# galatolofederico/clip-glass

Hardware: AMD Instinct MI355X
Metric: candidate latents scored/sec (GAN→CLIP fitness), StyleGAN2_ffhq_d pop=64 (higher is better)
Workload: dtype f16; 1 GPU; StyleGAN2_ffhq_d: StyleGAN2 config-f 1024px G+D + CLIP ViT-B/32, pop=64 per GPU, batch_size=4, n_obj=2; pop_per_gpu=64, global_pop=64, batch_size=4, parallelism=population-shard x1, device=AMD Radeon Graphics (gfx950:sramecc+:xnack-), 256 CUs, hbm_gib=288

## Files before the change

### clip_glass_amd/csrc/common.h

```cpp
#pragma once
#include <hip/hip_runtime.h>
#include <stdint.h>

#include <atomic>
#include <mutex>
#include <stdio.h>
#include <stdlib.h>

typedef _Float16 half_t;
typedef _Float16 h2 __attribute__((ext_vector_type(2)));
typedef _Float16 h4 __attribute__((ext_vector_type(4)));
typedef _Float16 h8 __attribute__((ext_vector_type(8)));
typedef float f4 __attribute__((ext_vector_type(4)));
typedef float f16x __attribute__((ext_vector_type(16)));

#define GLASS_SQRT2 1.41421356237309504880f

__device__ __forceinline__ f16x mfma32(h8 a, h8 b, f16x c) {
    return __builtin_amdgcn_mfma_f32_32x32x16_f16(a, b, c, 0, 0, 0);
}
__device__ __forceinline__ int mfma32_row(int reg, int lane) { return (reg & 3) + 8 * (reg >> 2) + 4 * (lane >> 5); }
__device__ __forceinline__ void philox4x32_10(uint32_t c[4], uint32_t k0, uint32_t k1) {
#pragma unroll
    for (int i = 0; i < 10; ++i) {
// ... 18 lines not shown
    const int my = oy >> 1, mx = ox >> 1;
    const float wy0 = (oy & 1) ? 0.25f : 0.75f, wx0 = (ox & 1) ? 0.25f : 0.75f;
    float s = 0.f;
    s += ((my >= 1 && mx >= 1) ? wy0 * wx0 : 0.f) * t[0];
    s += (my >= 1 ? wy0 * (1.f - wx0) : 0.f) * t[1];
    s += (mx >= 1 ? (1.f - wy0) * wx0 : 0.f) * t[2];
    s += (1.f - wy0) * (1.f - wx0) * t[3];
    return s;
}

struct DevOnce {
    std::atomic<bool> done[32] = {};
    static int dev() {
        int d = 0;
        if (hipGetDevice(&d) != hipSuccess || d < 0 || d >= 32) return -1;
        return d;
    }
    bool first() const {
        const int d = dev();
        return d < 0 || !done[d].load(std::memory_order_acquire);
    }
    void set() {
        const int d = dev();
        if (d >= 0) done[d].store(true, std::memory_order_release);
    }
    template <class F> void run(F&& setup) {
        if (first()) {
            setup();
            set();
        }
    }
};
struct GlassDevProps { int cus, lds_optin; };
inline GlassDevProps glass_dev_props() {
    static std::atomic<int> cus[32] = {}, lds[32] = {};
    int d = 0;
    if (hipGetDevice(&d) != hipSuccess || d < 0 || d >= 32) d = 0;
    if (!cus[d].load()) {
        hipDeviceProp_t prop;
        if (hipGetDeviceProperties(&prop, d) == hipSuccess) {
            lds[d].store((int)prop.sharedMemPerBlockOptin > 0 ? (int)prop.sharedMemPerBlockOptin : (int)prop.sharedMemPerBlock);
            cus[d].store(prop.multiProcessorCount);
        }
    }
    return GlassDevProps{cus[d].load() > 0 ? cus[d].load() : 256, lds[d].load() > 0 ? lds[d].load() : 64 * 1024};
}
inline int glass_cu_count() { return glass_dev_props().cus; }
inline bool glass_lds_fits(int bytes) {
    const GlassDevProps dp = glass_dev_props();
    if (bytes <= dp.lds_optin) return true;
    static std::mutex mu;
    static int seen_dev[16], seen_bytes[16], n_seen = 0;
    int d = 0;
    (void)hipGetDevice(&d);
    std::lock_guard<std::mutex> lk(mu);
    for (int i = 0; i < n_seen; ++i)
        if (seen_dev[i] == d && seen_bytes[i] == bytes) return false;
    if (n_seen == 16) return false;
    seen_dev[n_seen] = d;
    seen_bytes[n_seen++] = bytes;
    if (n_seen == 16) fprintf(stderr, "libglass: further LDS refusals are not reported\n");
    fprintf(stderr, "libglass: device %d offers %d B of opt-in LDS per workgroup; a kernel family that needs %d B is refused and its "
                    "layers fall back to a slower kernel (expected on gfx950: 163840 B)\n", d, dp.lds_optin, bytes);
    return false;
}

#define GLASS_NOMINAL_POP 64

__device__ __forceinline__ float lrelu_sqrt2(float v) { return (v > 0.f ? v : 0.2f * v) * GLASS_SQRT2; }
struct ActK { float k1, k2; };
__device__ __forceinline__ ActK act_consts(int act, float s) {
    return ActK{(act == 1 ? GLASS_SQRT2 : 1.f) * s, (act == 1 ? 0.2f * GLASS_SQRT2 : act == 2 ? 0.f : 1.f) * s};
}
__device__ __forceinline__ f4 act_apply(f4 v, ActK k) { return __builtin_elementwise_max(v * k.k1, v * k.k2); }

struct ConvParams {
    const half_t* x;
    long long x_bstride;
    int B, H, W, Cin;
    int Hc, Wc;
    int KS, stride, pad;
    const half_t* w;
    const half_t* w_up;
    long long w_bstride;
    int Neff, Cout;
    int up;
    int Ho, Wo;
    const float* sn;
    int sn_stride;
    const half_t* sn16;
    const half_t* pre_shift16;
    const float* pre_shift;
    int in_up;
    const float* dscale;
    int ds_stride;
    const float* noise;
    float noise_strength;
    int batch_size;
    const float* bias;
    const float* shift;
    int act;
    const half_t* res;
    int res_cs;
    int res_up;
    float out_scale;
    const float* rgb_y;
    const float* rgb_w;
    const float* rgb_b;
    half_t* rgb_x_out;
    half_t* rgb_xs_out;
    const float* trgb_w;
    const float* trgb_b;
    const float* trgb_sn;
    int trgb_sn_stride;
    const float* trgb_smax;
    int trgb_smax_stride;
    const float* trgb_yprev;
    float* trgb_yout;
    float* rgb_tanh_out;
    float* trgb_part;
    const half_t* trgb_tab;
    half_t* xs_out;
    const half_t* post_scale16;
    int post_stride;
    const half_t* skip_x;
    const half_t* skip_w;
    int dry_run;
    int x_planar32;
    int x_planar8;
    int y_planar8;
    int row_walk;
    half_t* y;
    float* y32;
};

struct GemmParams {
    const half_t* a;
    const half_t* w;
    int M, N, K;
    const float* bias;
    int mode;
    half_t* out16;
    float* out32;
    int ldo;
    int kpt;
    long long w_tap_stride;
    int batch;
    long long a_bs, w_bs, o_bs;
    int cand_rows;
    int cand_batch;
    int g_on, g_h, g_w, g_hc, g_wc, g_stride, g_pad, g_ks, g_cin;
    long long g_xbs;
    int ld;
};
```

### clip_glass_amd/csrc/engine.cpp

```cpp
#include "engine.h"

#include <math.h>
#include <string.h>

#include <algorithm>
#include <stdlib.h>

#include "kernels.h"

static thread_local std::string g_err;
void glass_set_error(const std::string& s) { g_err = s; }
extern "C" const char* glass_last_error(void) { return g_err.c_str(); }
extern "C" const char* glass_version(void) { return "clip-glass-amd 0.1 (gfx950)"; }

void glass_pack_conv(const float* W, int cout, int cin, int ks, int cin_pad, std::vector<_Float16>& out) {
    const float coef = 1.0f / sqrtf((float)cin * ks * ks);
    out.assign((size_t)ks * ks * cout * cin_pad, (_Float16)0.f);
    for (int o = 0; o < cout; ++o)
        for (int i = 0; i < cin; ++i)
            for (int t = 0; t < ks * ks; ++t)
                out[((size_t)t * cout + o) * cin_pad + i] = (_Float16)(W[((size_t)o * cin + i) * ks * ks + t] * coef);
}

int glass_fold_upconv(const float* W, int cout, int cin, std::vector<_Float16>& out) {
// ... 454 lines not shown
}

static int finalize_clip(glass_engine* e) {
    const glass_config& c = e->cfg;
    const int W = c.clip_width, ps = c.clip_patch, G = c.clip_res / ps, T = G * G + 1, E = c.clip_embed;
    const std::string v = "clip.visual.";
    GET(conv1, v + "conv1.weight");
    GET(cls, v + "class_embedding");
    GET(pos, v + "positional_embedding");
    GET(lg, v + "ln_pre.weight");
    GET(lb, v + "ln_pre.bias");
    GET(pg, v + "ln_post.weight");
    GET(pb, v + "ln_post.bias");
    GET(proj, v + "proj");
    REQUIRE(numel(conv1) == (size_t)W * 3 * ps * ps && numel(cls) == (size_t)W && numel(pos) == (size_t)T * W &&
                numel(proj) == (size_t)W * E,
            GLASS_ERR_ARG, "bad CLIP visual shapes");
    const int K = 3 * ps * ps, Kp = clip_patch_k(c);
    std::vector<_Float16> pw = to_half(conv1->data.data(), numel(conv1));
    if (Kp != K) {
        std::vector<_Float16> padded((size_t)W * Kp, (_Float16)0.f);
        for (int n = 0; n < W; ++n) std::copy(pw.begin() + (size_t)n * K, pw.begin() + (size_t)(n + 1) * K, padded.begin() + (size_t)n * Kp);
        pw.swap(padded);
    }
    int rc = upload(e, &e->c_patch_w, pw);
    if (rc) return rc;
    if ((rc = upload(e, &e->c_cls, cls->data))) return rc;
    if ((rc = upload(e, &e->c_pos, pos->data))) return rc;
    if ((rc = upload(e, &e->c_lnpre_g, lg->data))) return rc;
    if ((rc = upload(e, &e->c_lnpre_b, lb->data))) return rc;
    if ((rc = upload(e, &e->c_lnpost_g, pg->data))) return rc;
    if ((rc = upload(e, &e->c_lnpost_b, pb->data))) return rc;
    if ((rc = upload(e, &e->c_proj, proj->data))) return rc;
    int rc2 = load_clip_blocks(e, "clip.visual.transformer.resblocks.", c.clip_layers, W, e->cblk);
    if (rc2) return rc2;
    if (find(e, "clip.token_embedding.weight") != nullptr) {
        GET(tok, "clip.token_embedding.weight");
        GET(tpos, "clip.positional_embedding");
        GET(fg, "clip.ln_final.weight");
        GET(fb, "clip.ln_final.bias");
        GET(tp, "clip.text_projection");
        REQUIRE(tok->dims.size() == 2 && tpos->dims.size() == 2 && tpos->dims[1] == tok->dims[1], GLASS_ERR_ARG,
                "bad CLIP text embedding shapes");
        e->t_vocab = (int)tok->dims[0];
        e->t_width = (int)tok->dims[1];
        e->t_ctx = (int)tpos->dims[0];
        REQUIRE(e->t_width % 64 == 0 && numel(tp) == (size_t)e->t_width * E, GLASS_ERR_ARG, "bad CLIP text projection shape");
        int nl = 0;
        char nm2[256];
        for (;; ++nl) {
            snprintf(nm2, sizeof nm2, "clip.transformer.resblocks.%d.ln_1.weight", nl);
            if (!find(e, nm2)) break;
        }
        if ((rc = upload(e, &e->t_tok, tok->data))) return rc;
        if ((rc = upload(e, &e->t_pos, tpos->data))) return rc;
        if ((rc = upload(e, &e->t_lnf_g, fg->data))) return rc;
        if ((rc = upload(e, &e->t_lnf_b, fb->data))) return rc;
        if ((rc = upload(e, &e->t_proj, tp->data))) return rc;
        if ((rc = load_clip_blocks(e, "clip.transformer.resblocks.", nl, e->t_width, e->tblk))) return rc;
    }
    return GLASS_OK;
}

static int alloc_buffers(glass_engine* e) {
    const glass_config& c = e->cfg;
    const int P = c.max_pop, L = c.latent_size, CH = e->chunk;
    int rc;
    if ((rc = dev_alloc(e, &e->d_z, (size_t)P * L))) return rc;
    if ((rc = dev_alloc(e, &e->d_w0, (size_t)P * L))) return rc;
    if ((rc = dev_alloc(e, &e->d_w1, (size_t)P * L))) return rc;
    if ((rc = dev_alloc(e, &e->d_s, (size_t)P * e->S_total))) return rc;
    if ((rc = dev_alloc(e, &e->d_s16, (size_t)P * e->S_total))) return rc;
    if ((rc = dev_alloc(e, &e->d_smax, (size_t)P * e->n_style))) return rc;
    if ((rc = dev_alloc(e, &e->d_trgb_tab, (size_t)P * 32 * 512))) return rc;
    {
        size_t part = 0;
        for (int b = 0; b < c.n_blocks; ++b)
            if (c.channels[b] > 128 && c.channels[b] % 128 == 0 && c.channels[b] <= 512)
                part = std::max(part, (size_t)(c.channels[b] / 128) * (size_t)P * 3 * ((size_t)4 << b) * ((size_t)4 << b));
        if (part && (rc = dev_alloc(e, &e->d_trgb_part, part))) return rc;
    }
    if (e->cfg.generator != GLASS_GEN_BIGGAN_DEEP && e->cfg.n_blocks > 0) {
        int cmax = 16;
        for (int i = 0; i < e->cfg.n_blocks; ++i) cmax = std::max(cmax, (int)e->cfg.channels[i]);
        e->cap_a = 256LL * 9 * cmax;
        e->cap_c = 256LL * 4 * cmax;
        if ((rc = dev_alloc(e, &e->ws_a, (size_t)(e->cap_a * P)))) return rc;
        if ((rc = dev_alloc(e, &e->ws_c, (size_t)(e->cap_c * P)))) return rc;
        if (e->cfg.use_discriminator) {
            if ((rc = dev_alloc(e, &e->ws_a2, (size_t)(e->cap_a * P)))) return rc;
            if ((rc = dev_alloc(e, &e->ws_c2, (size_t)(e->cap_c * P)))) return rc;
        }
    } else if (e->cfg.generator == GLASS_GEN_BIGGAN_DEEP) {
        const int cmax = 4 * e->cfg.bg_ch;
        e->cap_a = 256LL * 9 * cmax;
        e->cap_c = 256LL * 4 * cmax;
        if ((rc = dev_alloc(e, &e->ws_a, (size_t)(e->cap_a * P)))) return rc;
        if ((rc = dev_alloc(e, &e->ws_c, (size_t)(e->cap_c * P)))) return rc;
    }
    if ((rc = dev_alloc(e, &e->d_epsrow, (size_t)P * e->n_style))) return rc;
    if ((rc = dev_alloc(e, &e->d_dscale, (size_t)P * e->D_total))) return rc;
    for (auto& g : e->gconv) {
        const bool fused_ok = g.up && g.cin % 32 == 0 && g.cout % 32 == 0 && g.res_in >= 16;
        const bool tiled_ok = !g.up && g.cin % 32 == 0 && g.cout % 32 == 0 && g.res_in % 32 == 0;
        g.welems = 9LL * g.cin * g.cout;
        g.premod = (fused_ok || tiled_ok) && g.welems * 2 <= (500LL << 10);
        if (g.premod && (rc = dev_alloc(e, &g.wm, (size_t)P * g.welems))) return rc;
    }
    if (c.noise_mode != 0) {
        const int n_mb = P / c.batch_size;
        for (auto& g : e->gconv) {
            float* p;
            if ((rc = dev_alloc(e, &p, (size_t)n_mb * g.res_out * g.res_out))) return rc;
            e->d_noise.push_back(p);
        }
    }
    size_t maxact = 0;
    for (int b = 0; b < c.n_blocks; ++b) {
        const size_t res = 4u << b;
        size_t ch = c.channels[b];
        if (b > 0) ch = std::max<size_t>(ch, c.channels[b - 1]);
        maxact = std::max(maxact, (res + 1) * (res + 1) * ch);
    }
    if (c.n_blocks > 0) maxact = std::max(maxact, (size_t)16 * (c.channels[0] + 16));
    e->act_elems = maxact * CH;
    for (int i = 0; i < 8 && c.n_blocks > 0; ++i)
        if (i >= 6 || c.use_discriminator)
            if ((rc = dev_alloc(e, &e->act[i], e->act_elems))) return rc;
    for (int i = 0; i < 4; ++i)
        if ((rc = dev_alloc(e, &e->ybuf[i], (size_t)CH * 3 * e->R * e->R))) return rc;
    if (c.n_blocks > 0) {
        e->n_low = 0;
        while (e->n_low < c.n_blocks && (4 << e->n_low) <= e->low_res) ++e->n_low;
        if (e->n_low < 1) e->n_low = 1;
        const size_t rl = 4u << (e->n_low - 1);
        size_t cmax = 16;
        for (int b = 0; b < e->n_low; ++b) cmax = std::max<size_t>(cmax, c.channels[b]);
        if (e->n_low < c.n_blocks) cmax = std::max<size_t>(cmax, c.channels[e->n_low]);
        const size_t low_elems = (size_t)P * (rl + 1) * (rl + 1) * (cmax + 16);
        const int n_lowbuf = c.use_discriminator ? 6 : 2;
        for (int i = 0; i < n_lowbuf; ++i)
            if ((rc = dev_alloc(e, &e->low[i], low_elems))) return rc;
        for (int i = 0; i < 2; ++i)
            if ((rc = dev_alloc(e, &e->ylow[i], (size_t)P * 3 * rl * rl))) return rc;
    }
    if ((rc = dev_alloc(e, &e->d_img, (size_t)CH * 3 * e->R * e->R))) return rc;
    const int W = c.clip_width, ps = c.clip_patch, G = c.clip_res / ps, T = G * G + 1;
    const size_t Kp = (size_t)clip_patch_k(c);
    if ((rc = dev_alloc(e, &e->d_patches, (size_t)P * G * G * Kp))) return rc;
    if (Kp != (size_t)3 * ps * ps) GLASS_HIP(hipMemset(e->d_patches, 0, (size_t)P * G * G * Kp * sizeof(half_t)));
    if ((rc = dev_alloc(e, &e->d_pe, (size_t)P * G * G * W))) return rc;
    if ((rc = dev_alloc(e, &e->d_x, (size_t)P * T * W))) return rc;
    if ((rc = dev_alloc(e, &e->d_ln16, (size_t)P * T * W))) return rc;
    if ((rc = dev_alloc(e, &e->d_qkv, (size_t)P * T * 3 * W))) return rc;
    if ((rc = dev_alloc(e, &e->d_attn, (size_t)P * T * W))) return rc;
    if ((rc = dev_alloc(e, &e->d_hid, (size_t)P * T * 4 * W))) return rc;
    if ((rc = dev_alloc(e, &e->d_cls, (size_t)P * W))) return rc;
    if ((rc = dev_alloc(e, &e->d_feat, (size_t)P * c.clip_embed))) return rc;
    if ((rc = dev_alloc(e, &e->d_sim, (size_t)P))) return rc;
    if ((rc = dev_alloc(e, &e->d_dis, (size_t)P))) return rc;
    if ((rc = dev_alloc(e, &e->d_F, (size_t)P * 2))) return rc;
    if ((rc = dev_alloc(e, &e->d_target, (size_t)c.clip_embed))) return rc;
    if (c.use_discriminator && c.n_blocks > 0) {
        if ((rc = dev_alloc(e, &e->d_dfin, (size_t)P * 16 * c.channels[0]))) return rc;
        if ((rc = dev_alloc(e, &e->d_dh, (size_t)P * c.channels[0]))) return rc;
        if ((rc = dev_alloc(e, &e->d_dh_part, (size_t)16 * P * c.channels[0]))) return rc;
    }
    {
        std::vector<DenseDesc> dd;
        for (auto& g : e->gconv) {
            DenseDesc q;
            q.x = e->d_s + g.style_off; q.ldx = e->S_total; q.K = g.cin; q.wt = g.wsq; q.N = g.cout; q.bias = nullptr;
            q.out = e->d_dscale + g.ds_off; q.ldo = e->D_total; q.eps_row = e->d_epsrow + g.style_idx; q.eps_stride = e->n_style;
            dd.push_back(q);
            e->demod_max_n = std::max(e->demod_max_n, g.cout);
        }
        DenseDesc* dptr = nullptr;
        if ((rc = upload(e, &dptr, dd))) return rc;
        e->d_demod_desc = dptr;
    }
    GLASS_HIP(hipMemset(e->d_dis, 0, (size_t)P * sizeof(float)));
    e->h_pinned_bytes = std::max((size_t)P * L, (size_t)P * (c.clip_embed + 8)) * sizeof(float);
    GLASS_HIP(hipHostMalloc((void**)&e->h_pinned, e->h_pinned_bytes, hipHostMallocDefault));
    return GLASS_OK;
}

static int finalize_gpt2(glass_engine* e) {
    if (!find(e, "gpt2.transformer.wte.weight")) return GLASS_OK;
    GET(wte, "gpt2.transformer.wte.weight");
    GET(wpe, "gpt2.transformer.wpe.weight");
    GET(lg, "gpt2.transformer.ln_f.weight");
    GET(lb, "gpt2.transformer.ln_f.bias");
    REQUIRE(wte->dims.size() == 2 && wpe->dims.size() == 2 && wpe->dims[1] == wte->dims[1], GLASS_ERR_ARG, "bad GPT-2 embedding shapes");
    e->g_vocab = (int)wte->dims[0];
    e->g_dim = (int)wte->dims[1];
    e->g_npos = (int)wpe->dims[0];
    const int D = e->g_dim;
    REQUIRE(D % 64 == 0, GLASS_ERR_ARG, "GPT-2 width must be a multiple of the 64-wide head");
    int rc;
    if ((rc = upload(e, &e->g_wte, wte->data))) return rc;
    if ((rc = upload(e, &e->g_wpe, wpe->data))) return rc;
    if ((rc = upload(e, &e->g_lnf_g, lg->data))) return rc;
    if ((rc = upload(e, &e->g_lnf_b, lb->data))) return rc;
    char nm[256];
    auto tr = [](const HostTensor* w, int nx, int nf) {
        std::vector<float> v((size_t)nx * nf);
        for (int i = 0; i < nx; ++i)
            for (int j = 0; j < nf; ++j) v[(size_t)j * nx + i] = w->data[(size_t)i * nf + j];
        return v;
    };
    for (int i = 0;; ++i) {
        snprintf(nm, sizeof nm, "gpt2.transformer.h.%d.", i);
        const std::string p = nm;
        if (!find(e, p + "ln_1.weight")) break;
        glass_engine::Gpt2Block b;
        GET(l1g, p + "ln_1.weight"); GET(l1b, p + "ln_1.bias"); GET(l2g, p + "ln_2.weight"); GET(l2b, p + "ln_2.bias");
        GET(wa, p + "attn.c_attn.weight"); GET(ba, p + "attn.c_attn.bias");
        GET(wo, p + "attn.c_proj.weight"); GET(bo, p + "attn.c_proj.bias");
        GET(wf, p + "mlp.c_fc.weight"); GET(bf, p + "mlp.c_fc.bias");
        GET(wp, p + "mlp.c_proj.weight"); GET(bp, p + "mlp.c_proj.bias");
        REQUIRE(numel(wa) == (size_t)3 * D * D && numel(wo) == (size_t)D * D && numel(wf) == (size_t)4 * D * D &&
                    numel(wp) == (size_t)4 * D * D, GLASS_ERR_ARG, "bad GPT-2 block shapes: " + p);
        if ((rc = upload(e, &b.ln1_g, l1g->data))) return rc;
        if ((rc = upload(e, &b.ln1_b, l1b->data))) return rc;
        if ((rc = upload(e, &b.ln2_g, l2g->data))) return rc;
        if ((rc = upload(e, &b.ln2_b, l2b->data))) return rc;
        if ((rc = upload(e, &b.w_qkv, tr(wa, D, 3 * D)))) return rc;
        if ((rc = upload(e, &b.b_qkv, ba->data))) return rc;
        if ((rc = upload(e, &b.w_o, tr(wo, D, D)))) return rc;
        if ((rc = upload(e, &b.b_o, bo->data))) return rc;
        if ((rc = upload(e, &b.w_fc, tr(wf, D, 4 * D)))) return rc;
        if ((rc = upload(e, &b.b_fc, bf->data))) return rc;
        if ((rc = upload(e, &b.w_pr, tr(wp, 4 * D, D)))) return rc;
        if ((rc = upload(e, &b.b_pr, bp->data))) return rc;
        e->gblk.push_back(b);
    }
    return GLASS_OK;
}

extern "C" int glass_engine_finalize(glass_engine* e) {
    REQUIRE(e, GLASS_ERR_ARG, "null engine");
    REQUIRE(!e->finalized, GLASS_ERR_STATE, "engine already finalized");
    GLASS_HIP(hipSetDevice(e->cfg.device));
    int rc = GLASS_OK;
    if (e->cfg.n_blocks > 0) {
        if ((rc = finalize_generator(e))) return rc;
        if (e->cfg.use_discriminator && (rc = finalize_discriminator(e))) return rc;
    }
    if (e->cfg.generator == GLASS_GEN_BIGGAN_DEEP && (rc = glass_biggan_finalize(e))) return rc;
    if ((rc = finalize_gpt2(e))) return rc;
    if ((rc = finalize_clip(e))) return rc;
    if ((rc = alloc_buffers(e))) return rc;
    e->host.clear();
    e->finalized = true;
    return GLASS_OK;
}

extern "C" int glass_engine_set_target(glass_engine* e, const float* feat, int32_t n) {
    REQUIRE(e && feat, GLASS_ERR_ARG, "null argument");
    REQUIRE(e->finalized, GLASS_ERR_STATE, "finalize() first");
    REQUIRE(n == e->cfg.clip_embed, GLASS_ERR_ARG, "target feature length != clip_embed");
    GLASS_HIP(hipSetDevice(e->cfg.device));
    GLASS_HIP(hipMemcpy(e->d_target, feat, (size_t)n * sizeof(float), hipMemcpyHostToDevice));
    e->has_target = true;
    return GLASS_OK;
}

void collect_profile(glass_engine* e) {
    std::map<std::string, glass_prof_row> rows;
    std::vector<std::string> order;
    for (auto& pe : e->prof_events) {
        float ms = 0.f;
        hipEventElapsedTime(&ms, pe.e0, pe.e1);
        auto it = rows.find(pe.name);
        if (it == rows.end()) {
            glass_prof_row r;
            memset(&r, 0, sizeof r);
            strncpy(r.name, pe.name.c_str(), sizeof(r.name) - 1);
            it = rows.emplace(pe.name, r).first;
            order.push_back(pe.name);
        }
        it->second.launches += 1;
        it->second.total_ms += ms;
        it->second.flops += pe.flops;
        it->second.bytes += pe.bytes;
    }
    e->prof_rows.clear();
    for (auto& n : order) e->prof_rows.push_back(rows[n]);
    e->prof_events.clear();
    e->event_next = 0;
}

void run_conv(glass_engine* e, const ConvParams& p, const char* tag, double flops, double bytes) {
    if (!(p.out_scale > 0.f)) {
        if (e->launch_error.empty()) e->launch_error = std::string("out_scale must be positive: ") + tag;
        return;
    }
    Prof pr(e, tag, flops, bytes);
    const char* k = p.up ? launch_upconv_fused(p, e->cur) : nullptr;
    if (p.rgb_tanh_out) {
        k = launch_conv_tiled(p, e->cur);
        if (!k && e->launch_error.empty()) e->launch_error = std::string("no kernel writes the planar tanh output of layer ") + tag;
        if (!k) k = "(refused)";
        if (pr.on) pr.pe.name = std::string(tag) + "@" + k;
        if (e->profiling) e->tag_kernel[tag] = k;
        return;
// ... 288 lines not shown
                if (e->profiling) e->tag_kernel[tag] = k;
                std::swap(X, O);
                continue;
            }
            pr.on = false;
        }
        const bool fuse_down = conv_down_supported(r, d.cin, d.cout);
        if (i == 0 && rgb_y) {
            ConvParams q = p;
            q.rgb_y = rgb_y; q.rgb_w = e->d_frgb_w; q.rgb_b = e->d_frgb_b;
            q.rgb_x_out = fuse_down ? nullptr : X;
            q.rgb_xs_out = fuse_down ? XS : nullptr;
            snprintf(tag, sizeof tag, "D.fromrgb+conv0.r%d.%dx%d", r, d.cin, d.cin);
            const double px = (double)B * r * r;
            Prof pr(e, tag, 2.0 * px * (9.0 * d.cin * d.cin + 3.0 * d.cin), px * (12.0 + 2.0 * d.cin + (fuse_down ? 0.5 : 2.0) * d.cin));
            const char* k = launch_conv_stream(q, e->cur);
            if (k) {
                fused_rgb = true;
                have_xs = fuse_down;
                if (pr.on) pr.pe.name = std::string(tag) + "@" + k;
                if (e->profiling) e->tag_kernel[tag] = k;
            } else {
                pr.on = false;
            }
        }
        if (i == 0 && rgb_y && !fused_rgb) run_fromrgb(e, B, rgb_y, X);
        snprintf(tag, sizeof tag, "D.conv0.r%d.%dx%d", r, d.cin, d.cin);
        if (!fused_rgb) {
            ConvParams qx = p;
            qx.xs_out = XS; qx.dry_run = 1;
            if (!have_xs &&(launch_conv_glds(qx, e->cur) || launch_conv_tiled(qx, e->cur))) {
                qx.dry_run = 0;
                p = qx;
                have_xs = true;
            }
            run_conv(e, p, tag, 2.0 * B * (double)r * r * 9 * d.cin * d.cin, 4.0 * B * (double)r * r * d.cin + (have_xs ? 0.5 * B * (double)r * r * d.cin : 0.0));
        }
        if (!have_xs && x_was_planar && e->launch_error.empty()) e->launch_error = std::string("chunk-planar block input without the fused blur-down: ") + tag;
        if (!have_xs) {
            snprintf(tag, sizeof tag, "D.blurdown.r%d", r);
            Prof pr(e, tag, 2.0 * B * (double)r2 * r2 * d.cin * 16, 2.5 * B * (double)r * r * d.cin);
            launch_blur_down(X, B, r, r, d.cin, XS, e->cur);
        }
        if (fuse_down) {
            snprintf(tag, sizeof tag, "D.down.r%d.%dx%d", r2, d.cin, d.cout);
            const double px2 = (double)B * r2 * r2;
            Prof pr(e, tag, 2.0 * px2 * (9.0 + 1.0) * d.cin * d.cout, 2.0 * (B * (double)r * r * d.cin + px2 * (d.cin + d.cout)));
            const char* k = launch_conv_down(Hb, XS, d.w1, d.wskip, d.b1, O, B, r, d.cin, d.cout, e->cur);
            if (k) {
                if (pr.on) pr.pe.name = std::string(tag) + "@" + k;
                if (e->profiling) e->tag_kernel[tag] = k;
                std::swap(X, O);
                continue;
            }
            pr.on = false;
        }
        ConvParams q = conv_defaults();
        q.x = HB; q.x_bstride = (long long)(r + 1) * (r + 1) * d.cin; q.B = B; q.H = q.W = r + 1; q.Cin = d.cin;
        q.Hc = q.Wc = r2; q.KS = 3; q.stride = 2; q.pad = 0; q.w = d.w1; q.Cout = q.Neff = d.cout; q.Ho = q.Wo = r2;
        q.bias = d.b1; q.act = 1; q.out_scale = 0.70710678118654752440f; q.y = O;
        bool hb_planar = false;
        {
            ConvParams qp = q;
            qp.skip_x = XS; qp.skip_w = d.wskip; qp.x_planar32 = 1; qp.dry_run = 1;
            hb_planar = blur_pad2_planar32_ok(d.cin) && launch_conv_s2(qp, e->cur) != nullptr;
        }
        {
            snprintf(tag, sizeof tag, "D.blur.r%d", r);
            Prof pr(e, tag, 2.0 * B * (double)(r + 1) * (r + 1) * d.cin * 16, 4.0 * B * (double)r * r * d.cin);
            launch_blur_pad2(Hb, B, r, r, d.cin, HB, e->cur, hb_planar);
        }
        snprintf(tag, sizeof tag, "D.conv1.r%d.%dx%d", r2, d.cin, d.cout);
        const double f1 = 2.0 * B * (double)r2 * r2 * 9 * d.cin * d.cout, fs = 2.0 * B * (double)r2 * r2 * d.cin * d.cout;
        {
            ConvParams qs = q;
            qs.skip_x = XS; qs.skip_w = d.wskip; qs.dry_run = 1;
            qs.x_planar32 = hb_planar;
            if (hb_planar ? launch_conv_s2(qs, e->cur) : launch_conv_tiled(qs, e->cur)) {
                qs.dry_run = 0;
                Prof pr(e, tag, f1 + fs, 2.0 * B * ((double)(r + 1) * (r + 1) * d.cin + (double)r2 * r2 * (d.cin + d.cout)));
                const char* k = hb_planar ? launch_conv_s2(qs, e->cur) : launch_conv_tiled(qs, e->cur);
                if (pr.on) pr.pe.name = std::string(tag) + "@" + k;
                if (e->profiling) e->tag_kernel[tag] = k;
                std::swap(X, O);
                continue;
            }
        }
        ConvParams s = conv_defaults();
        s.x = XS; s.x_bstride = (long long)r2 * r2 * d.cin; s.B = B; s.H = s.W = r2; s.Cin = d.cin;
        s.Hc = s.Wc = r2; s.KS = 1; s.pad = 0; s.w = d.wskip; s.Cout = s.Neff = d.cout; s.Ho = s.Wo = r2; s.y = S;
        char stag[64];
        snprintf(stag, sizeof stag, "D.skip.r%d.%dx%d", r2, d.cin, d.cout);
        run_conv(e, s, stag, fs, 2.0 * B * (double)r2 * r2 * (d.cin + d.cout));
        q.res = S;
        run_conv(e, q, tag, f1, 2.0 * B * ((double)(r + 1) * (r + 1) * d.cin + 2.0 * r2 * r2 * d.cout));
        std::swap(X, O);
    }
    return X;
}

static void run_fromrgb(glass_engine* e, int B, const float* y, half_t* X) {
    const glass_config& c = e->cfg;
    const int n = c.n_blocks;
    Prof pr(e, "D.fromrgb", 2.0 * B * (double)e->R * e->R * 3 * c.channels[n - 1],
            B * (double)e->R * e->R * (12.0 + 2.0 * c.channels[n - 1]));
    launch_fromrgb(y, B, e->R, c.channels[n - 1], e->d_frgb_w, e->d_frgb_b, X, e->cur);
}

static void run_d_head(glass_engine* e, int P, const half_t* X, half_t* scratch) {
    const glass_config& c = e->cfg;
    const int CL = c.channels[0];
    {
        Prof pr(e, "D.mbstd", 0, 4.0 * P * 16 * CL);
        launch_mbstd(X, P, 16, CL, e->d_final_cpad, c.batch_size, c.mbstd_group, 1e-8f, scratch, e->cur);
    }
    ConvParams p = conv_defaults();
    p.x = scratch; p.x_bstride = 16LL * e->d_final_cpad; p.B = P; p.H = p.W = 4; p.Cin = e->d_final_cpad; p.Hc = p.Wc = 4;
    p.KS = 3; p.pad = 1; p.w = e->d_final_w; p.Cout = p.Neff = CL; p.Ho = p.Wo = 4; p.bias = e->d_final_b; p.act = 1;
    p.y = e->d_dfin;
    run_conv(e, p, "D.final_conv", 2.0 * P * 16 * 9.0 * (CL + 1) * CL, 2.0 * 9 * CL * (CL + 1));
    GemmParams g;
    memset(&g, 0, sizeof g);
    g.a = e->d_dfin; g.w = e->d_dense0_w; g.M = P; g.N = CL; g.K = 16 * CL; g.bias = e->d_dense0_b; g.mode = 4;
    g.out32 = e->d_dh; g.ldo = CL; g.cand_rows = 1;
    const int S0 = 16;
    if (e->d_dh_part && g.K % (S0 * 64) == 0 && P <= e->cfg.max_pop) {
        GemmParams q = g;
        q.ld = g.K; q.K = g.K / S0; q.batch = S0; q.a_bs = q.K; q.w_bs = q.K; q.o_bs = (long long)P * CL;
        q.bias = nullptr; q.mode = 3; q.out32 = e->d_dh_part;
        Prof pr(e, "D.dense0", 2.0 * P * (double)g.K * CL, 2.0 * (double)g.K * CL);
        const char* k = launch_gemm_tiled(q, e->cur);
        if (k) {
            launch_dense01_finish(e->d_dh_part, S0, q.o_bs, g.bias, e->d_dense1_wt, e->d_dense1_b, e->d_dis, P, CL, e->cur);
            if (pr.on) pr.pe.name = std::string("D.dense0+1@") + k + "+dense01_finish";
            return;
        }
        pr.on = false;
    }
    run_gemm(e, g, "D.dense0");
    {
        Prof pr(e, "D.dense1", 2.0 * P * CL, 0);
        launch_dense(e->d_dh, CL, P, CL, e->d_dense1_wt, 1, e->d_dense1_b, e->d_dis, 1, 0, 0, nullptr, 0, e->cur);
    }
}

void run_clip(glass_engine* e, int P, int l0, int l1);
static void run_clip_rest(glass_engine* e, int P, int l0) {
    if (l0 == 0) {
        run_clip(e, P, -1, 1 << 20);
        return;
    }
    run_clip(e, P, l0, 1 << 20);
}
void run_clip(glass_engine* e, int P, int l0, int l1) {
    const glass_config& c = e->cfg;
    const int W = c.clip_width, ps = c.clip_patch, G = c.clip_res / ps, T = G * G + 1, M = P * T;
    GemmParams g;
    if (l0 == 0) {
        memset(&g, 0, sizeof g);
        g.a = e->d_patches; g.w = e->c_patch_w; g.M = P * G * G; g.N = W; g.K = clip_patch_k(c); g.mode = 3; g.out32 = e->d_pe; g.ldo = W; g.cand_rows = G * G;
        run_gemm(e, g, "clip.patch_embed");
        Prof pr(e, "clip.embed_lnpre", 0, 8.0 * M * W);
        launch_embed_lnpre(e->d_pe, e->c_cls, e->c_pos, e->c_lnpre_g, e->c_lnpre_b, P, T, W, e->d_x, e->cur);
    }
    for (int li = l0 < 0 ? 0 : l0; li < l1 && li < (int)e->cblk.size(); ++li) {
        auto& b = e->cblk[li];
        {
            Prof pr(e, "clip.layernorm", 0, 6.0 * M * W);
            launch_layernorm(e->d_x, W, M, W, b.ln1_g, b.ln1_b, e->d_ln16, nullptr, e->cur);
        }
        memset(&g, 0, sizeof g);
        g.a = e->d_ln16; g.w = b.w_qkv; g.M = M; g.N = 3 * W; g.K = W; g.bias = b.b_qkv; g.mode = 0; g.out16 = e->d_qkv; g.ldo = 3 * W; g.cand_rows = T;
        run_gemm(e, g, "clip.qkv");
        {
            Prof pr(e, "clip.attention", 4.0 * P * c.clip_heads * (double)T * T * 64, 8.0 * M * W);
            launch_attention(e->d_qkv, P, T, c.clip_heads, 64, 0, e->d_attn, e->cur);
        }
        memset(&g, 0, sizeof g);
        g.a = e->d_attn; g.w = b.w_out; g.M = M; g.N = W; g.K = W; g.bias = b.b_out; g.mode = 2; g.out32 = e->d_x; g.ldo = W; g.cand_rows = T;
        run_gemm(e, g, "clip.attn_out");
        {
            Prof pr(e, "clip.layernorm", 0, 6.0 * M * W);
            launch_layernorm(e->d_x, W, M, W, b.ln2_g, b.ln2_b, e->d_ln16, nullptr, e->cur);
        }
        memset(&g, 0, sizeof g);
        g.a = e->d_ln16; g.w = b.w_fc; g.M = M; g.N = 4 * W; g.K = W; g.bias = b.b_fc; g.mode = 1; g.out16 = e->d_hid; g.ldo = 4 * W; g.cand_rows = T;
        run_gemm(e, g, "clip.mlp_fc");
        memset(&g, 0, sizeof g);
        g.a = e->d_hid; g.w = b.w_proj; g.M = M; g.N = W; g.K = 4 * W; g.bias = b.b_proj; g.mode = 2; g.out32 = e->d_x; g.ldo = W; g.cand_rows = T;
        run_gemm(e, g, "clip.mlp_proj");
    }
    if (l1 >= (int)e->cblk.size()) {
        Prof pr(e, "clip.head", 2.0 * P * W * c.clip_embed, 4.0 * W * c.clip_embed);
        launch_layernorm(e->d_x, (long long)T * W, P, W, e->c_lnpost_g, e->c_lnpost_b, nullptr, e->d_cls, e->cur);
        launch_dense(e->d_cls, W, P, W, e->c_proj, c.clip_embed, nullptr, e->d_feat, c.clip_embed, 0, 0, nullptr, 0,
                     e->cur);
        launch_cosine(e->d_feat, e->d_target, P, c.clip_embed, e->d_sim, e->cur);
    }
}

static int run_pass(glass_engine* e, const float* latents, int P, int generation, int first_mb,
                    const glass_noise* noise, float* out_F, float* images) {
    REQUIRE(e && latents, GLASS_ERR_ARG, "null argument");
    REQUIRE(e->finalized, GLASS_ERR_STATE, "finalize() first (weights not loaded)");
    const glass_config& c = e->cfg;
    REQUIRE(P > 0 && P <= c.max_pop, GLASS_ERR_ARG, "population size out of range (max_pop)");
    REQUIRE(P % c.batch_size == 0, GLASS_ERR_ARG,
            "population size must be a multiple of batch_size (reference asserts: models.py:112)");
    const bool biggan = c.generator == GLASS_GEN_BIGGAN_DEEP;
    REQUIRE(e->cfg.n_blocks > 0 || biggan, GLASS_ERR_STATE, "this engine was created without a GAN (n_blocks = 0)");
    if (out_F) REQUIRE(e->has_target, GLASS_ERR_STATE, "set_target() first");
    GLASS_HIP(hipSetDevice(c.device));
    e->launch_error.clear();
    const int L = c.latent_size;
    memcpy(e->h_pinned, latents, (size_t)P * L * sizeof(float));
    GLASS_HIP(hipEventRecord(e->ev0, e->cur));
    GLASS_HIP(hipMemcpyAsync(e->d_z, e->h_pinned, (size_t)P * L * sizeof(float), hipMemcpyHostToDevice, e->cur));
    const int ps = c.clip_patch, G = c.clip_res / ps;
    const size_t img_elems = (size_t)3 * e->R * e->R;
    if (biggan) {
        int rc = glass_biggan_prepare(e, P);
        if (rc) return rc;
        for (int c0 = 0; c0 < P; c0 += e->chunk) {
            const int B = std::min(e->chunk, P - c0);
            float* y = e->ybuf[0];
            if ((rc = glass_biggan_chunk(e, c0, B, y))) return rc;
            if (images) {
                launch_finalize_image(y, e->d_img, (long long)B * img_elems, e->cur);
                GLASS_HIP(hipMemcpyAsync(images + (size_t)c0 * img_elems, e->d_img, (size_t)B * img_elems * sizeof(float),
                                         hipMemcpyDeviceToHost, e->cur));
            }
            if (out_F) {
                Prof pr(e, "clip.resize", 0, B * (16.0 * c.clip_res * c.clip_res * 3 + 2.0 * 3 * c.clip_res * c.clip_res));
                launch_resize_patches(y, B, e->R, c.clip_res, ps, clip_patch_k(c), e->d_patches + (size_t)c0 * G * G * clip_patch_k(c), e->cur);
            }
        }
        if (out_F) {
            run_clip(e, P, 0, 1 << 20);
            launch_assemble_F(e->d_sim, e->d_dis, P, c.n_obj, e->d_F, e->cur);
            GLASS_HIP(hipMemcpyAsync(e->h_pinned, e->d_F, (size_t)P * c.n_obj * sizeof(float), hipMemcpyDeviceToHost, e->cur));
        }
        GLASS_HIP(hipEventRecord(e->ev1, e->cur));
        GLASS_HIP(hipStreamSynchronize(e->cur));
        GLASS_HIP(hipGetLastError());
        GLASS_HIP(hipEventElapsedTime(&e->last_ms, e->ev0, e->ev1));
        if (out_F) memcpy(out_F, e->h_pinned, (size_t)P * c.n_obj * sizeof(float));
        e->last_P = P;
        if (e->profiling) collect_profile(e);
        return GLASS_OK;
    }
    const bool noise_ov = e->clip_overlap && c.noise_mode == 1;
    int rc;
    if (noise_ov) {
        e->cur = e->stream_d;
        rc = upload_noise(e, P, generation, first_mb, noise);
        e->cur = e->stream;
        if (rc) return rc;
        GLASS_HIP(hipEventRecord(e->ev_noise, e->stream_d));
        run_styles(e, P);
        GLASS_HIP(hipStreamWaitEvent(e->stream, e->ev_noise, 0));
    } else {
        run_styles(e, P);
        rc = upload_noise(e, P, generation, first_mb, noise);
        if (rc) return rc;
    }
    const bool want_d = out_F && c.use_discriminator && c.n_obj == 2;
    const int n = c.n_blocks;
    const int nlow = std::min(n, e->n_low);
    const int nd = (int)e->dblk.size();
    const int d_hi = want_d ? std::max(0, n - nlow) : 0;
    const half_t* xlow = nullptr;
    const float* ylow = nullptr;
    {
        half_t* const pp[2] = {e->low[0], e->low[1]};
        float* const yb[2] = {e->ylow[0], e->ylow[1]};
        run_g_blocks(e, 0, P, 0, nlow, e->g_const, 0, pp, nullptr, yb, &xlow, &ylow);
    }
    const int res_low = 4 << (nlow - 1);
    const long long xlow_bs = (long long)res_low * res_low * c.channels[nlow - 1];
    half_t* dmid = e->low[5];
    const int res_mid = d_hi < nd ? e->dblk[d_hi].res : 4;
    const long long dmid_bs = (long long)res_mid * res_mid * (d_hi < nd ? e->dblk[d_hi].cin : c.channels[0]);
    const int n_chunks = (P + e->chunk - 1) / e->chunk;
    while ((int)e->ev_g.size() < n_chunks) {
        hipEvent_t a, b2;
        GLASS_HIP(hipEventCreateWithFlags(&a, hipEventDisableTiming));
        GLASS_HIP(hipEventCreateWithFlags(&b2, hipEventDisableTiming));
        e->ev_g.push_back(a);
        e->ev_d.push_back(b2);
    }
    const bool overlap = e->overlap && out_F;
    const bool clip_ov = e->clip_overlap && !overlap && out_F && want_d;
    hipStream_t sd = overlap ? e->stream_d : e->stream;
    for (int c0 = 0, k = 0; c0 < P; c0 += e->chunk, ++k) {
        const int B = std::min(e->chunk, P - c0);
        const int set = k & 1;
        e->cur = e->stream;
        if (overlap && k >= 2) GLASS_HIP(hipStreamWaitEvent(e->stream, e->ev_d[k - 2], 0));
        const float* y = ylow + (size_t)c0 * 3 * res_low * res_low;
        if (nlow < n) {
            half_t* const pp[2] = {e->act[6], e->act[7]};
            float* const yb[2] = {e->ybuf[2 * set], e->ybuf[2 * set + 1]};
            const half_t* xo;
            run_g_blocks(e, c0, B, nlow, n, xlow + (size_t)c0 * xlow_bs, xlow_bs, pp, y, yb, &xo, &y);
        }
        if (images) {
            launch_finalize_image(y, e->d_img, (long long)B * img_elems, e->cur);
            GLASS_HIP(hipMemcpyAsync(images + (size_t)c0 * img_elems, e->d_img, (size_t)B * img_elems * sizeof(float),
                                     hipMemcpyDeviceToHost, e->cur));
        }
        if (out_F) {
            if (overlap) {
                GLASS_HIP(hipEventRecord(e->ev_g[k], e->stream));
                GLASS_HIP(hipStreamWaitEvent(sd, e->ev_g[k], 0));
            }
            e->cur = sd;
            {
                Prof pr(e, "clip.resize", 0, B * (16.0 * c.clip_res * c.clip_res * 3 + 2.0 * 3 * c.clip_res * c.clip_res));
                launch_resize_patches(y, B, e->R, c.clip_res, ps, clip_patch_k(c), e->d_patches + (size_t)c0 * G * G * clip_patch_k(c),
                                      e->cur);
            }
            if (clip_ov && c0 + e->chunk >= P) {
                run_clip(e, P, 0, GLASS_CLIP_SERIAL_LAYERS);
                GLASS_HIP(hipEventRecord(e->ev_g[0], e->stream));
                GLASS_HIP(hipStreamWaitEvent(e->stream_d, e->ev_g[0], 0));
                e->cur = e->stream_d;
                run_clip_rest(e, P, GLASS_CLIP_SERIAL_LAYERS);
                GLASS_HIP(hipEventRecord(e->ev_d[0], e->stream_d));
                e->cur = e->stream;
            }
            if (want_d) {
                if (d_hi > 0) {
                    half_t* const bufs[5] = {e->act[1], e->act[2], e->act[3], e->act[4], e->act[5]};
                    half_t* Xo = run_d_blocks(e, B, 0, d_hi, e->act[0], bufs, y);
                    GLASS_HIP(hipMemcpyAsync(dmid + (size_t)c0 * dmid_bs, Xo, (size_t)B * dmid_bs * sizeof(half_t),
                                             hipMemcpyDeviceToDevice, e->cur));
                } else {
                    run_fromrgb(e, B, y, dmid + (size_t)c0 * dmid_bs);
                }
            }
            if (overlap) GLASS_HIP(hipEventRecord(e->ev_d[k], sd));
        }
    }
    if (want_d) {
        e->cur = sd;
        half_t* const bufs[5] = {e->low[0], e->low[1], e->low[2], e->low[3], e->low[4]};
        half_t* Xo = run_d_blocks(e, P, d_hi, nd, dmid, bufs);
        run_d_head(e, P, Xo, Xo == e->low[0] ? e->low[1] : e->low[0]);
    }
    if (out_F) {
// ... 469 lines not shown
```

### clip_glass_amd/csrc/engine.h

```cpp
#pragma once
#include <hip/hip_runtime.h>

#include <algorithm>
#include <map>
#include <string>
#include <vector>

#include "../../include/glass.h"
#include "common.h"

void glass_set_error(const std::string& s);
#define GLASS_HIP(call)                                                                        \
    do {                                                                                       \
        hipError_t _e = (call);                                                                \
        if (_e != hipSuccess) {                                                                \
            glass_set_error(std::string(#call) + " failed: " + hipGetErrorString(_e) + " at " + \
                            __FILE__ + ":" + std::to_string(__LINE__));                        \
            return GLASS_ERR_HIP;                                                              \
        }                                                                                      \
    } while (0)

struct HostTensor {
    std::vector<int64_t> dims;
    std::vector<float> data;
};

struct GConv {
    int cin, cout, res_in, res_out, up;
    int style_idx, style_off, ds_off, noise_idx;
    half_t* w = nullptr;
    half_t* w_up = nullptr;
    half_t* wm = nullptr;
    long long welems = 0;
    bool premod = false;
    float* wsq = nullptr;
    float* bias = nullptr;
    float noise_strength = 0.f;
};
struct GRgb {
    int cin, res, style_idx, style_off;
    float* w = nullptr;
    float* bias = nullptr;
};
struct DBlock {
    int cin, cout, res;
    half_t *w0 = nullptr, *w1 = nullptr, *wskip = nullptr;
    float *b0 = nullptr, *b1 = nullptr;
};
struct ClipBlock {
    float *ln1_g, *ln1_b, *ln2_g, *ln2_b;
    half_t *w_qkv, *w_out, *w_fc, *w_proj;
    float *b_qkv, *b_out, *b_fc, *b_proj;
};

struct BgBlock {
    int cin, cout, mid, up, res_in;
    int bn_off[4];
    half_t* w[4] = {nullptr, nullptr, nullptr, nullptr};
    float* b3 = nullptr;
};
struct BgState {
    int R = 0, Ctot = 0, zd = 0, nc = 0, c0 = 0;
    float *et = nullptr, *genz_wt = nullptr, *genz_b = nullptr;
    float *bn_wt = nullptr, *bn_bias = nullptr, *bn_inv_std = nullptr, *bn_mean = nullptr, *bn_prebias = nullptr;
    std::vector<BgBlock> blocks;
    int attn_before = -1, attn_C = 0, attn_res = 0;
    half_t *attn_w_tpg = nullptr, *attn_w_o = nullptr;
    int final_bn_off = 0, rgb_cpad = 32;
    half_t* rgb_w = nullptr;
    float* rgb_b = nullptr;
    half_t* tab16 = nullptr;
    float *cond = nullptr, *tab = nullptr, *h32 = nullptr, *a_S = nullptr;
    half_t *x[2] = {nullptr, nullptr}, *t1 = nullptr, *t2 = nullptr, *t3 = nullptr;
    half_t *a_T = nullptr, *a_theta = nullptr, *a_phi = nullptr, *a_gT = nullptr, *a_P = nullptr, *a_O = nullptr;
};
int glass_biggan_finalize(glass_engine* e);
int glass_biggan_prepare(glass_engine* e, int P);
int glass_biggan_chunk(glass_engine* e, int c0, int B, float* y);

struct ProfEvent {
    std::string name;
    double flops, bytes;
    hipEvent_t e0, e1;
};

struct glass_engine {
    glass_config cfg;
    int R = 0;
    int n_style = 0;
    int S_total = 0, D_total = 0;
    int chunk = 0;
    bool finalized = false, has_target = false;
    hipStream_t stream = nullptr, stream_d = nullptr, cur = nullptr;
    bool overlap = false, clip_overlap = false;
    std::vector<hipEvent_t> ev_g, ev_d;
    hipEvent_t ev0 = nullptr, ev1 = nullptr, ev_noise = nullptr;
    float last_ms = 0.f;
    int last_P = 0;
    std::string launch_error;

    std::map<std::string, HostTensor> host;
    std::vector<void*> allocs;

    std::vector<float*> map_wt, map_b;
    float *style_wt = nullptr, *style_b = nullptr;
    int *d_style_off = nullptr, *d_style_len = nullptr;
    std::vector<int> style_off, style_len;
    half_t* g_const = nullptr;
    void* d_demod_desc = nullptr;
    int demod_max_n = 0;
    std::vector<GConv> gconv;
    std::vector<GRgb> grgb;
    BgState bg;
    float *d_frgb_w = nullptr, *d_frgb_b = nullptr;
    std::vector<DBlock> dblk;
    half_t* d_final_w = nullptr;
    float* d_final_b = nullptr;
    int d_final_cpad = 0;
    half_t* d_dense0_w = nullptr;
    float *d_dense0_b = nullptr, *d_dense1_wt = nullptr, *d_dense1_b = nullptr;
    half_t* c_patch_w = nullptr;
    float *c_cls = nullptr, *c_pos = nullptr, *c_lnpre_g = nullptr, *c_lnpre_b = nullptr;
    float *c_lnpost_g = nullptr, *c_lnpost_b = nullptr, *c_proj = nullptr;
    std::vector<ClipBlock> cblk;
    struct Gpt2Block { float *ln1_g, *ln1_b, *ln2_g, *ln2_b, *w_qkv, *b_qkv, *w_o, *b_o, *w_fc, *b_fc, *w_pr, *b_pr; };
    std::vector<Gpt2Block> gblk;
    float *g_wte = nullptr, *g_wpe = nullptr, *g_lnf_g = nullptr, *g_lnf_b = nullptr;
    int g_vocab = 0, g_dim = 0, g_npos = 0;
    struct Gpt2Work {
        int P = 0, nctx = 0, length = 0;
        int *d_tok = nullptr, *d_gen = nullptr, *d_state = nullptr, *d_samp = nullptr;
        int sample = 0;
        float *x = nullptr, *ln = nullptr, *qkv = nullptr, *att = nullptr, *hid = nullptr, *last = nullptr, *logits = nullptr,
              *kc = nullptr, *vc = nullptr, *part = nullptr, *stats = nullptr, *pairs = nullptr, *pst = nullptr;
        size_t part_elems = 0;
        hipGraph_t graph = nullptr;
        hipGraphExec_t exec = nullptr;
        float last_ms = 0.f;
    } gwork, gwork_alt;
    std::vector<ClipBlock> tblk;
    float *t_tok = nullptr, *t_pos = nullptr, *t_lnf_g = nullptr, *t_lnf_b = nullptr, *t_proj = nullptr;
    struct TextWork {
        int n_texts = 0;
        int *d_tok = nullptr, *d_rows = nullptr;
        float *x = nullptr, *cls = nullptr, *feat = nullptr;
        half_t *ln16 = nullptr, *qkv = nullptr, *att = nullptr, *hid = nullptr;
    } twork;
    int t_width = 0, t_ctx = 0, t_vocab = 0;
    float* d_target = nullptr;

    half_t* d_s16 = nullptr;
    half_t* ws_a = nullptr;
    float* ws_c = nullptr;
    half_t* ws_a2 = nullptr;
    float* ws_c2 = nullptr;
    long long cap_a = 0, cap_c = 0;
    half_t* d_trgb_tab = nullptr;
    float* d_trgb_part = nullptr;
    float *d_z = nullptr, *d_w0 = nullptr, *d_w1 = nullptr, *d_s = nullptr, *d_smax = nullptr, *d_epsrow = nullptr,
          *d_dscale = nullptr;
    std::vector<float*> d_noise;
    half_t* act[8] = {nullptr, nullptr, nullptr, nullptr, nullptr, nullptr, nullptr, nullptr};
    half_t* low[6] = {nullptr, nullptr, nullptr, nullptr, nullptr, nullptr};
    float* ylow[2] = {nullptr, nullptr};
    int low_res = 32, n_low = 0;
    size_t act_elems = 0;
    float* ybuf[4] = {nullptr, nullptr, nullptr, nullptr};
    float* d_img = nullptr;
    half_t *d_patches = nullptr, *d_ln16 = nullptr, *d_qkv = nullptr, *d_attn = nullptr, *d_hid = nullptr;
    float *d_pe = nullptr, *d_x = nullptr, *d_cls = nullptr, *d_feat = nullptr, *d_sim = nullptr, *d_dis = nullptr,
          *d_F = nullptr, *d_dh = nullptr, *d_dh_part = nullptr;
    half_t* d_dfin = nullptr;
    float* h_pinned = nullptr;
    size_t h_pinned_bytes = 0;

    int bg_tap = -2;
    std::vector<float> bg_tap_data;
    int bg_tap_dims[4] = {0, 0, 0, 0};
    bool profiling = false;
    std::string prof_filter;
    std::map<std::string, std::string> tag_kernel;
    std::vector<ProfEvent> prof_events;
    std::vector<glass_prof_row> prof_rows;
    std::vector<hipEvent_t> event_pool;
    size_t event_next = 0;
};

#define REQUIRE(cond, code, msg)          \
    do {                                  \
        if (!(cond)) {                    \
            glass_set_error(msg);         \
            return code;                  \
        }                                 \
    } while (0)

template <typename T>
inline int dev_alloc(glass_engine* e, T** p, size_t n) {
    void* q = nullptr;
    hipError_t err = hipMalloc(&q, std::max<size_t>(n, 1) * sizeof(T));
    if (err != hipSuccess) {
        glass_set_error(std::string("hipMalloc failed: ") + hipGetErrorString(err));
        return GLASS_ERR_NOMEM;
    }
    e->allocs.push_back(q);
    *p = (T*)q;
    return GLASS_OK;
}
template <typename T>
inline int upload(glass_engine* e, T** p, const std::vector<T>& v) {
    int rc = dev_alloc(e, p, v.size());
    if (rc) return rc;
    GLASS_HIP(hipMemcpy(*p, v.data(), v.size() * sizeof(T), hipMemcpyHostToDevice));
    return GLASS_OK;
}

inline const HostTensor* find(glass_engine* e, const std::string& name) {
    auto it = e->host.find(name);
    return it == e->host.end() ? nullptr : &it->second;
}
#define GET(var, name)                                                            \
    const HostTensor* var = find(e, name);                                        \
    REQUIRE(var != nullptr, GLASS_ERR_STATE, std::string("missing tensor: ") + (name))

inline size_t numel(const HostTensor* t) {
    size_t n = 1;
    for (auto d : t->dims) n *= (size_t)d;
    return n;
}

struct Prof {
    glass_engine* e;
    bool on;
    ProfEvent pe;
    Prof(glass_engine* e_, const char* name, double flops, double bytes) : e(e_), on(e_->profiling) {
        if (on && !e->prof_filter.empty()) {
            auto it = e->tag_kernel.find(name);
            on = it != e->tag_kernel.end() && it->second.find(e->prof_filter) != std::string::npos;
        }
        if (!on) return;
        auto get = [&]() {
            if (e->event_next == e->event_pool.size()) {
                hipEvent_t ev;
                hipEventCreate(&ev);
                e->event_pool.push_back(ev);
            }
            return e->event_pool[e->event_next++];
        };
        pe.name = name;
        pe.flops = flops;
        pe.bytes = bytes;
        pe.e0 = get();
        pe.e1 = get();
        hipEventRecord(pe.e0, e->cur);
    }
    ~Prof() {
        if (!on) return;
        hipEventRecord(pe.e1, e->cur);
        e->prof_events.push_back(pe);
    }
};

void collect_profile(glass_engine* e);
void run_conv(glass_engine* e, const ConvParams& p, const char* tag, double flops, double bytes);
void run_gemm(glass_engine* e, const GemmParams& p, const char* tag);
ConvParams conv_defaults();
void run_clip(glass_engine* e, int P, int l0, int l1);
#define GLASS_CLIP_SERIAL_LAYERS 1
std::vector<_Float16> to_half(const float* p, size_t n, float scale = 1.f);
std::vector<float> scaled(const float* p, size_t n, float scale);
std::vector<float> transposed(const float* W, int N, int K, float coef);

int glass_fold_upconv(const float* W, int cout, int cin, std::vector<_Float16>& out);
void glass_pack_conv(const float* W, int cout, int cin, int ks, int cin_pad, std::vector<_Float16>& out);
```

### clip_glass_amd/csrc/gemm_tiled.hip

```cpp
#include "common.h"
#include "kernels.h"
#include <stdlib.h>

#define GROWB 144

template <int BN, bool GATHER = false>
__global__ __launch_bounds__(256, 2) void gemm_tiled_kernel(GemmParams p) {
    if (p.batch > 1) {
        p.a += (long long)blockIdx.z * p.a_bs;
        p.w += (long long)blockIdx.z * p.w_bs;
        if (p.out16) p.out16 += (long long)blockIdx.z * p.o_bs;
        if (p.out32) p.out32 += (long long)blockIdx.z * p.o_bs;
    }
    constexpr int NJ = BN / 64;
    constexpr int NVA = 128 * 8, NVB = BN * 8;
    constexpr int NA = NVA / 256, NB = NVB / 256;
    __shared__ __attribute__((aligned(16))) char smem[(128 + BN) * GROWB];
    char* As = smem;
    char* Bs = smem + 128 * GROWB;
    const int t = threadIdx.x, lane = t & 63, wave = t >> 6;
    const int lr = lane & 31, kh = lane >> 5;
    const int wm = wave >> 1, wn = wave & 1;
    const int gy = p.N / BN, n_tiles = ((p.M + 127) >> 7) * gy;
    const int per_xcd = (n_tiles + 7) >> 3;
    const int tile = (blockIdx.x & 7) * per_xcd + (blockIdx.x >> 3);
    if (tile >= min(((int)(blockIdx.x & 7) + 1) * per_xcd, n_tiles)) return;
    const int m0 = (tile / gy) * 128, n0 = (tile % gy) * BN;
    const int part = t & 7;

    h8 ra[NA], rb[NB];
    long long gbase[GATHER ? NA : 1];
    int giy[GATHER ? NA : 1], gix[GATHER ? NA : 1], okm = 0;
    if (GATHER) {
#pragma unroll
        for (int k = 0; k < NA; ++k) {
            const int row = min(m0 + (t >> 3) + 32 * k, p.M - 1), hw = p.g_hc * p.g_wc;
            const int b = row / hw, rem = row - b * hw, oy = rem / p.g_wc, ox = rem - oy * p.g_wc;
            giy[k] = oy * p.g_stride - p.g_pad;
            gix[k] = ox * p.g_stride - p.g_pad;
            gbase[k] = (long long)b * p.g_xbs + ((long long)giy[k] * p.g_w + gix[k]) * p.g_cin + part * 8;
        }
    }
    auto load = [&](int k0) {
        const int kw = k0 + ((p.kpt && p.ld) ? (int)blockIdx.z * p.K : 0);
        if (GATHER) {
            const int tap = kw / p.g_cin, ci = kw - tap * p.g_cin, ty = tap / p.g_ks, tx = tap - ty * p.g_ks;
            const long long toff = ((long long)ty * p.g_w + tx) * p.g_cin + ci;
            okm = 0;
#pragma unroll
            for (int k = 0; k < NA; ++k) {
                const bool ok = (unsigned)(giy[k] + ty) < (unsigned)p.g_h && (unsigned)(gix[k] + tx) < (unsigned)p.g_w;
                ra[k] = *(const h8*)(p.a + (ok ? gbase[k] + toff : (long long)part * 8));
                okm |= (ok ? 1 : 0) << k;
            }
        } else {
#pragma unroll
        for (int k = 0; k < NA; ++k) {
            const int row = min(m0 + (t >> 3) + 32 * k, p.M - 1);
            ra[k] = *(const h8*)(p.a + (long long)row * (p.ld ? p.ld : p.K) + k0 + part * 8);
        }
        }
        const int rs = p.kpt ? p.kpt : (p.ld ? p.ld : p.K);
        const half_t* wk = p.kpt ? p.w + (long long)(kw / p.kpt) * p.w_tap_stride + (kw % p.kpt) : p.w + k0;
#pragma unroll
        for (int k = 0; k < NB; ++k) {
            const int row = (t >> 3) + 32 * k;
            rb[k] = *(const h8*)(wk + (long long)(n0 + row) * rs + part * 8);
        }
    };
    auto store = [&]() {
        const h8 zero = {0, 0, 0, 0, 0, 0, 0, 0};
#pragma unroll
        for (int k = 0; k < NA; ++k) *(h8*)(As + ((t >> 3) + 32 * k) * GROWB + part * 16) = (!GATHER || ((okm >> k) & 1)) ? ra[k] : zero;
#pragma unroll
        for (int k = 0; k < NB; ++k) *(h8*)(Bs + ((t >> 3) + 32 * k) * GROWB + part * 16) = rb[k];
    };

    f16x acc[2][NJ];
#pragma unroll
    for (int i = 0; i < 2; ++i)
#pragma unroll
        for (int j = 0; j < NJ; ++j)
#pragma unroll
            for (int q = 0; q < 16; ++q) acc[i][j][q] = 0.f;

    load(0);
    for (int k0 = 0; k0 < p.K; k0 += 64) {
        if (k0 > 0) __syncthreads();
        store();
        __syncthreads();
        if (k0 + 64 < p.K) load(k0 + 64);
#pragma unroll
        for (int kk = 0; kk < 4; ++kk) {
            h8 wf[NJ], xf[2];
#pragma unroll
            for (int j = 0; j < NJ; ++j)
                wf[j] = *(const h8*)(Bs + (wn * (BN / 2) + j * 32 + lr) * GROWB + kk * 32 + kh * 16);
#pragma unroll
            for (int i = 0; i < 2; ++i)
                xf[i] = *(const h8*)(As + (wm * 64 + i * 32 + lr) * GROWB + kk * 32 + kh * 16);
#pragma unroll
            for (int i = 0; i < 2; ++i)
#pragma unroll
                for (int j = 0; j < NJ; ++j) acc[i][j] = mfma32(wf[j], xf[i], acc[i][j]);
        }
    }
    f4 bq[NJ][4];
#pragma unroll
    for (int j = 0; j < NJ; ++j)
#pragma unroll
        for (int g = 0; g < 4; ++g) {
            bq[j][g] = f4{0.f, 0.f, 0.f, 0.f};
            if (p.bias) bq[j][g] = *(const f4*)(p.bias + n0 + wn * (BN / 2) + j * 32 + 8 * g + 4 * kh);
        }
#pragma unroll
    for (int i = 0; i < 2; ++i) {
        const int m = m0 + wm * 64 + i * 32 + lr;
        const int mc = min(m, p.M - 1);
        f4 rq[NJ][4];
        if (p.mode == 2) {
#pragma unroll
            for (int j = 0; j < NJ; ++j)
#pragma unroll
                for (int g = 0; g < 4; ++g)
                    rq[j][g] = *(const f4*)(p.out32 + (long long)mc * p.ldo + n0 + wn * (BN / 2) + j * 32 + 8 * g + 4 * kh);
        }
        if (m >= p.M) continue;
#pragma unroll
        for (int j = 0; j < NJ; ++j) {
#pragma unroll
            for (int g = 0; g < 4; ++g) {
                const int n = n0 + wn * (BN / 2) + j * 32 + 8 * g + 4 * kh;
                float v[4];
#pragma unroll
                for (int q = 0; q < 4; ++q) v[q] = acc[i][j][g * 4 + q] + bq[j][g][q];
                const long long oi = (long long)m * p.ldo + n;
                if (p.mode <= 1) {
                    h4 o;
#pragma unroll
                    for (int q = 0; q < 4; ++q)
                        o[q] = (half_t)(p.mode == 1 ? v[q] * __builtin_amdgcn_rcpf(1.f + __expf(-1.702f * v[q])) : v[q]);
                    *(h4*)(p.out16 + oi) = o;
                } else {
                    f4 o;
                    if (p.mode == 2) {
#pragma unroll
                        for (int q = 0; q < 4; ++q) o[q] = rq[j][g][q] + v[q];
                    } else {
#pragma unroll
                        for (int q = 0; q < 4; ++q) o[q] = p.mode == 4 ? lrelu_sqrt2(v[q]) : v[q];
                    }
                    *(f4*)(p.out32 + oi) = o;
                }
            }
        }
    }
}

const char* launch_gemm_tiled(const GemmParams& p, hipStream_t st) {
    if (p.K % 64 != 0 || p.ldo % 4 != 0 || (p.M < 64 && !p.kpt) || (p.kpt && p.kpt % 64 != 0)) return nullptr;
    const unsigned gx = (unsigned)((p.M + 127) / 128), gz = p.batch > 1 ? p.batch : 1;
    const long long gx_n = p.cand_rows ? ((long long)p.cand_rows * GLASS_NOMINAL_POP + 127) / 128 : gx;
    const long long gz_n = p.cand_batch ? GLASS_NOMINAL_POP : gz;
    const bool fills = gx_n * (p.N / 128) * gz_n >= 256;
    if (p.g_on && (!p.kpt || p.kpt != p.g_cin || p.g_cin % 64 != 0)) return nullptr;
    if (p.N % 128 == 0 && fills) {
        if (p.g_on) {
            hipLaunchKernelGGL((gemm_tiled_kernel<128, true>), dim3(8 * ((gx * (p.N / 128) + 7) / 8), 1, gz), dim3(256), 0, st, p);
            return "gemm_tiled_kernel<128,true>";
        }
        hipLaunchKernelGGL(gemm_tiled_kernel<128>, dim3(8 * ((gx * (p.N / 128) + 7) / 8), 1, gz), dim3(256), 0, st, p);
        return "gemm_tiled_kernel<128>";
    }
    if (p.N % 64 == 0) {
        if (p.g_on) {
            hipLaunchKernelGGL((gemm_tiled_kernel<64, true>), dim3(8 * ((gx * (p.N / 64) + 7) / 8), 1, gz), dim3(256), 0, st, p);
            return "gemm_tiled_kernel<64,true>";
        }
        hipLaunchKernelGGL(gemm_tiled_kernel<64>, dim3(8 * ((gx * (p.N / 64) + 7) / 8), 1, gz), dim3(256), 0, st, p);
        return "gemm_tiled_kernel<64>";
    }
    return nullptr;
}
```

### clip_glass_amd/csrc/kernels.h

```cpp
#pragma once
#include "common.h"

const char* launch_conv_direct(const ConvParams& p, hipStream_t st);
const char* launch_gemm_direct(const GemmParams& p, hipStream_t st);
const char* launch_conv_tiled(const ConvParams& p, hipStream_t st);
const char* launch_gemm_tiled(const GemmParams& p, hipStream_t st);
const char* launch_conv_stream(const ConvParams& p, hipStream_t st);
const char* launch_conv_gemm(const ConvParams& p, half_t* ws_a, long long cap_a, float* ws_c, long long cap_c, hipStream_t st);
bool conv_stream_applies(const ConvParams& p);
const char* launch_conv_glds(const ConvParams& p, hipStream_t st);
const char* launch_conv_wreg(const ConvParams& p, hipStream_t st);
bool conv_wreg_supported(int Cin, int Cout, int H, int W);
const char* launch_conv_s2(const ConvParams& p, hipStream_t st, bool force = false);
const char* launch_conv_down(const half_t* h, const half_t* xs, const half_t* w1, const half_t* ws, const float* b1, half_t* y,
                             int B, int R, int Cin, int Cout, hipStream_t st);
bool conv_down_supported(int R, int Cin, int Cout);
const char* launch_dblock0(const float* rgb_y, const float* rgb_w, const float* rgb_b, const half_t* w0, const float* b0, const half_t* w1,
                           const half_t* ws, const float* b1, half_t* y, int B, int R, int Cin, int Cout, hipStream_t st, int y_planar8 = 0);
bool dblock0_supported(int R, int Cin, int Cout);
const char* launch_upconv_fused(const ConvParams& p, hipStream_t st);

void launch_pixelnorm(const float* z, float* out, int P, int L, float eps, hipStream_t st);
void launch_dense01_finish(const float* part, int S, long long slab, const float* bias0, const float* w1, const float* b1, float* out, int P, int N,
                           hipStream_t st);
void launch_dense_splitk(const float* x, int ldx, int P, int K, const float* wt, int N, const float* bias, float* out, int ldo,
                         int mode, hipStream_t st);
void launch_dense(const float* x, int ldx, int P, int K, const float* wt, int N, const float* bias,
                  float* out, int ldo, int in_sq, int mode, const float* eps_row, int eps_stride,
                  hipStream_t st);
bool launch_mapping_fused(const float* z, float* out, int P, int L, float eps, const float* const* wt, const float* const* b, int n_layers,
                          hipStream_t st);
struct DenseDesc {
    const float* x; int ldx; int K; const float* wt; int N; const float* bias; float* out; int ldo;
    const float* eps_row; int eps_stride;
};
void launch_dense_multi(const DenseDesc* d_desc, int n_desc, int max_N, int P, int in_sq, int mode, hipStream_t st);
void launch_style_norm(float* s, int ld, int P, int n_layers, const int* d_off, const int* d_len,
                       float* smax, float* eps_row, float eps, hipStream_t st);
void launch_modulate_weights(const half_t* w, long long elems, int Cin, int Cout, const float* sn, int sn_stride,
                              const float* dscale, int ds_stride, int P, half_t* wm, hipStream_t st);
void launch_noise(float* out, int n_mb, int hw, uint32_t layer, uint32_t mb0, uint32_t generation,
                  uint64_t seed, hipStream_t st);

void launch_trgb_tables(const float* wrgb, const float* sn, int sn_stride, const float* smax, int smax_stride, int B, int NT,
                        half_t* tab, hipStream_t st);
void launch_trgb_finish(const float* part, int ntn, int B, int R, const float* bias, const float* yprev, float* yout, hipStream_t st);
bool launch_torgb(const half_t* x, int B, int H, int W, int C, const float* wrgb, const float* bias,
                  const float* sn, int sn_stride, const float* smax, int smax_stride,
                  const float* yprev, float* yout, hipStream_t st);
void launch_finalize_image(const float* y, float* img, long long n, hipStream_t st);
void launch_resize_patches(const float* y, int B, int R, int clip_res, int ps, int ld, half_t* patches,
                           hipStream_t st);
void launch_fromrgb(const float* y, int B, int R, int Cout, const float* w, const float* bias,
                    half_t* out, hipStream_t st);
void launch_blur_pad2(const half_t* x, int B, int H, int W, int C, half_t* out, hipStream_t st, int planar32 = 0);
bool blur_pad2_planar32_ok(int C);
void launch_blur_down(const half_t* x, int B, int H, int W, int C, half_t* out, hipStream_t st);
void launch_mbstd(const half_t* x, int B, int hw, int C, int Cpad, int batch_size, int group, float eps,
                  half_t* out, hipStream_t st);

void launch_embed_lnpre(const float* patch_emb, const float* cls, const float* pos, const float* g,
                        const float* b, int P, int T, int D, float* x, hipStream_t st);
void launch_embed_text(const int* tokens, const float* tok_emb, const float* pos, int n_rows, int ctx, int D, float* x,
                       hipStream_t st);
void launch_layernorm(const float* x, long long row_stride, int M, int D, const float* g, const float* b,
                      half_t* out16, float* out32, hipStream_t st);
void launch_layernorm_rows(const float* x, const int* rows, int M, int D, const float* g, const float* b, float* out32, hipStream_t st);
void launch_attention(const half_t* qkv, int n_img, int L, int heads, int hd, int causal, half_t* out,
                      hipStream_t st);
void launch_cosine(const float* feat, const float* target, int P, int D, float* sim, hipStream_t st);
void launch_assemble_F(const float* sim, const float* dis, int P, int n_obj, float* F, hipStream_t st);

void launch_bg_cond(const float* x, int P, int L, int zd, int nc, const float* et, float* cond, hipStream_t st);
void launch_bg_bn_tables(float* tab, int P, int C, const float* inv_std, const float* mean, const float* prebias,
                         hipStream_t st);
void launch_bg_to_half(const float* x, half_t* y, long long n, hipStream_t st);
void launch_bg_attn_split(const half_t* T, int B, int H, int W, int c8, int c2, half_t* theta, half_t* phi, half_t* gT,
                          hipStream_t st);
void launch_bg_softmax(const float* S, long long rows, int n, half_t* Pm, hipStream_t st);
void launch_bg_rgb_tanh(const half_t* x, int B, long long hw, int C, float* y, hipStream_t st);

struct BgTailParams {
    const half_t* h;
    const half_t* x0;
    const half_t* w3;
    const float* b3;
    const float* tab;
    int bnf_off, ctot;
    const half_t* rgb_w;
    int cpad;
    const float* rgb_b;
    float* y;
    int B, R;
};
bool bg_tail_supported(int R, int mid, int cout, int cin, int up, int cpad);
bool launch_bg_tail(const BgTailParams& p, hipStream_t st);
void launch_gpt2_embed(const int* tok, const float* wte, const float* wpe, int rows, int L, int pos0, int D, float* x,
                       hipStream_t st);
void launch_gemm_f32(const float* A, const float* W, const float* bias, float* out, int M, int N, int K, int lda, int ldo,
                     int mode, hipStream_t st, float* part = nullptr, size_t part_elems = 0, bool prefill = false);
bool gemm_f32_step_supported(int M, int K, int lda, bool ln_fused);
int launch_gemm_f32_step(const float* A, const float* W, const float* bias, float* out, int M, int N, int K, int lda, int ldo, int mode,
                         hipStream_t st, float* part, size_t part_elems, const float* stats, const float* lng, const float* lnb);
bool gpt2_head_supported(int M, int N, int K, int lda);
bool launch_gpt2_head_tail(const float* A, const float* W, int M, int N, int K, int lda, const float* stats_in, const float* lng, const float* lnb,
                           float* pairs, int* gen, int* state, const float* wte, const float* wpe, float* x, float* stats_out, hipStream_t st);
bool launch_gpt2_head(const float* A, const float* W, int M, int N, int K, int lda, const float* stats, const float* lng, const float* lnb,
                      float* logits, float* pairs, int* out, const int* step_dev, hipStream_t st);
void launch_gpt2_reduce(const float* part, int S, const float* bias, float* out, int M, int N, int ldo, int mode, hipStream_t st);
void launch_gpt2_finalize(const float* part, int S, const float* bias, float* x, int M, int D, float* stats, hipStream_t st);
#define GPT2_ATTENTION_LDS_MAX (160 * 1024)
size_t gpt2_attention_lds_bytes(int nd, int ns);
void launch_gpt2_attention(const float* qkv, float* kc, float* vc, int P, int nd, int past, int Tmax, int heads,
                           float* out, hipStream_t st, const int* past_dev = nullptr);
void launch_gpt2_attention_step(const float* qkv, const float* part, int S, const float* bias, float* kc, float* vc, int P, int Tmax, int heads,
                                float* out, hipStream_t st, const int* past_dev);
void launch_argmax(const float* logits, int rows, int N, int* out, hipStream_t st, const int* step_dev = nullptr, float* scratch = nullptr);
void launch_gpt2_embed_step(const int* gen, const int* state, int P, const float* wte, const float* wpe, int D, float* x, hipStream_t st,
                            float* stats = nullptr, bool partial_fmt = false);
bool gemm_f32_rowblk_supported(int M, int N, int K, int lda, bool ln_fused, bool stats_out);
bool launch_gemm_f32_rowblk(const float* A, const float* W, const float* bias, float* out, int M, int N, int K, int lda, int ldo, int mode,
                            hipStream_t st, const float* pst_in, int np_in, const float* lng, const float* lnb, float* pst_out);
void launch_gpt2_advance(int* state, hipStream_t st);
enum { GPT2_SP_SEED_LO, GPT2_SP_SEED_HI, GPT2_SP_GEN, GPT2_SP_ROW0, GPT2_SP_PURPOSE, GPT2_SP_TEMP, GPT2_SP_TOPK, GPT2_SP_STEP, GPT2_SP_WORDS };
#define GPT2_SAMPLE_TOPK_MAX 256
bool gpt2_sample_supported(int V);
void launch_gpt2_sample(const float* logits, int rows, int V, const int* sp, int* out, int* state, hipStream_t st);
bool launch_gpt2_head_sample(const float* A, const float* W, int M, int N, int K, int lda, const float* stats_in, const float* lng, const float* lnb,
                             float* logits, float* pairs, const int* sp, int* gen, int* state, bool tail, const float* wte, const float* wpe, float* x,
                             float* stats_out, hipStream_t st);
void launch_image_patches(const float* img, int n, int S, int ps, int ld, half_t* patches, hipStream_t st);
```

### clip_glass_amd/csrc/kernels_clip.hip

```cpp
#include "common.h"
#include "kernels.h"
#include <stdlib.h>

__device__ __forceinline__ float wsum(float v) {
#pragma unroll
    for (int o = 32; o > 0; o >>= 1) v += __shfl_xor(v, o);
    return v;
}

template <typename LoadF>
__device__ __forceinline__ void ln_row(LoadF load, int D, const float* g, const float* b, half_t* o16, float* o32) {
    const int lane = threadIdx.x & 63;
    if (D <= 1024) {
        float v[16];
#pragma unroll
        for (int k = 0; k < 16; ++k) v[k] = lane + 64 * k < D ? load(lane + 64 * k) : 0.f;
        float s = 0.f;
#pragma unroll
        for (int k = 0; k < 16; ++k) s += v[k];
        const float mean = wsum(s) / (float)D;
        float q = 0.f;
#pragma unroll
        for (int k = 0; k < 16; ++k) { const float d = lane + 64 * k < D ? v[k] - mean : 0.f; q += d * d; }
        const float rstd = rsqrtf(wsum(q) / (float)D + 1e-5f);
#pragma unroll
        for (int k = 0; k < 16; ++k) {
            const int i = lane + 64 * k;
            if (i < D) {
                const float o = (v[k] - mean) * rstd * g[i] + b[i];
                if (o16) o16[i] = (half_t)o;
                if (o32) o32[i] = o;
            }
        }
        return;
    }
    float s = 0.f;
    for (int i = lane; i < D; i += 64) s += load(i);
    const float mean = wsum(s) / (float)D;
    float q = 0.f;
    for (int i = lane; i < D; i += 64) { const float d = load(i) - mean; q += d * d; }
    const float rstd = rsqrtf(wsum(q) / (float)D + 1e-5f);
    for (int i = lane; i < D; i += 64) {
        const float v = (load(i) - mean) * rstd * g[i] + b[i];
        if (o16) o16[i] = (half_t)v;
        if (o32) o32[i] = v;
    }
}

__global__ __launch_bounds__(256) void embed_lnpre_kernel(const float* pe, const float* cls, const float* pos,
                                                          const float* g, const float* b, int P, int T, int D,
                                                          float* x) {
    const int row = blockIdx.x * 4 + (threadIdx.x >> 6);
    if (row >= P * T) return;
    const int p = row / T, t = row - p * T;
    const float* src = t == 0 ? cls : pe + ((long long)p * (T - 1) + (t - 1)) * D;
    const float* ps = pos + (long long)t * D;
    ln_row([&](int i) { return src[i] + ps[i]; }, D, g, b, nullptr, x + (long long)row * D);
}
void launch_embed_lnpre(const float* patch_emb, const float* cls, const float* pos, const float* g,
                        const float* b, int P, int T, int D, float* x, hipStream_t st) {
    hipLaunchKernelGGL(embed_lnpre_kernel, dim3((P * T + 3) / 4), dim3(256), 0, st, patch_emb, cls, pos, g, b, P,
                       T, D, x);
}

__global__ void embed_text_kernel(const int* tokens, const float* tok_emb, const float* pos, int ctx, int D, float* x) {
    const int row = blockIdx.x;
    const float* te = tok_emb + (long long)tokens[row] * D;
    const float* pe = pos + (long long)(row % ctx) * D;
    for (int i = threadIdx.x; i < D; i += blockDim.x) x[(long long)row * D + i] = te[i] + pe[i];
}
void launch_embed_text(const int* tokens, const float* tok_emb, const float* pos, int n_rows, int ctx, int D, float* x,
                       hipStream_t st) {
    hipLaunchKernelGGL(embed_text_kernel, dim3(n_rows), dim3(128), 0, st, tokens, tok_emb, pos, ctx, D, x);
}

__global__ __launch_bounds__(256) void layernorm_kernel(const float* x, long long row_stride, int M, int D,
                                                        const float* g, const float* b, half_t* o16, float* o32) {
    const int row = blockIdx.x * 4 + (threadIdx.x >> 6);
    if (row >= M) return;
    const float* xr = x + (long long)row * row_stride;
    ln_row([&](int i) { return xr[i]; }, D, g, b, o16 ? o16 + (long long)row * D : nullptr,
           o32 ? o32 + (long long)row * D : nullptr);
}
void launch_layernorm(const float* x, long long row_stride, int M, int D, const float* g, const float* b,
                      half_t* out16, float* out32, hipStream_t st) {
    hipLaunchKernelGGL(layernorm_kernel, dim3((M + 3) / 4), dim3(256), 0, st, x, row_stride, M, D, g, b, out16,
                       out32);
}

__global__ __launch_bounds__(256) void layernorm_rows_kernel(const float* x, const int* rows, int M, int D, const float* g, const float* b, float* o32) {
    const int m = blockIdx.x * 4 + (threadIdx.x >> 6);
    if (m >= M) return;
    const float* xr = x + (long long)rows[m] * D;
    ln_row([&](int i) { return xr[i]; }, D, g, b, nullptr, o32 + (long long)m * D);
}
void launch_layernorm_rows(const float* x, const int* rows, int M, int D, const float* g, const float* b, float* out32, hipStream_t st) {
    hipLaunchKernelGGL(layernorm_rows_kernel, dim3((M + 3) / 4), dim3(256), 0, st, x, rows, M, D, g, b, out32);
}

template <int NKB>
__global__ __launch_bounds__(256) void attention_mfma_kernel(const half_t* qkv, int L, int heads, int n_pairs, int causal,
                                                             half_t* out) {
    constexpr int PP = NKB == 2 ? 2 : 1;
    constexpr int WP = 4 / PP;
    constexpr int VROW = NKB * 64 + 16;
    __shared__ __attribute__((aligned(16))) char vts[PP][64 * VROW];
    const int t = threadIdx.x, lane = t & 63, wave = t >> 6, lr = lane & 31, kh = lane >> 5;
    const int pair = blockIdx.x * PP + wave / WP, qb = wave % WP;
    const int pc = min(pair, n_pairs - 1);
    const int img = pc / heads, h = pc - img * heads, D = heads * 64;
    const half_t* base = qkv + (long long)img * L * 3 * D + h * 64;
    const long long ts = 3LL * D;
    const int query = qb * 32 + lr;
    const bool qwave = qb < NKB;
    h8 qf[4], kf[NKB][4];
    if (qwave) {
        const half_t* qp = base + min(query, L - 1) * ts + kh * 8;
#pragma unroll
        for (int kk = 0; kk < 4; ++kk) qf[kk] = *(const h8*)(qp + kk * 16);
#pragma unroll
        for (int kb = 0; kb < NKB; ++kb) {
            const half_t* kp = base + min(kb * 32 + lr, L - 1) * ts + D + kh * 8;
#pragma unroll
            for (int kk = 0; kk < 4; ++kk) kf[kb][kk] = *(const h8*)(kp + kk * 16);
        }
    }
    constexpr int TP = 64 * WP;
    constexpr int NV = NKB * 32 * 8 / TP;
    const int pt = t % TP;
    h8 vv[NV];
#pragma unroll
    for (int u = 0; u < NV; ++u) {
        const int e = pt + TP * u, tok = e >> 3, d8 = e & 7;
        vv[u] = *(const h8*)(base + min(tok, L - 1) * ts + 2 * D + d8 * 8);
    }
    char* vt = vts[wave / WP];
#pragma unroll
    for (int u = 0; u < NV; ++u) {
        const int e = pt + TP * u, tok = e >> 3, d8 = e & 7;
        const int r = tok & 31, g = r >> 3;
        const int pos = ((tok >> 5) * 2 + (g >> 1)) * 16 + ((r >> 2) & 1) * 8 + (g & 1) * 4 + (r & 3);
#pragma unroll
        for (int j = 0; j < 8; ++j) *(half_t*)(vt + (d8 * 8 + j) * VROW + pos * 2) = tok < L ? vv[u][j] : (half_t)0.f;
    }
    f16x s[NKB];
    float inv = 0.f;
    if (qwave) {
#pragma unroll
        for (int kb = 0; kb < NKB; ++kb) {
#pragma unroll
            for (int r = 0; r < 16; ++r) s[kb][r] = 0.f;
#pragma unroll
            for (int kk = 0; kk < 4; ++kk) s[kb] = mfma32(kf[kb][kk], qf[kk], s[kb]);
        }
        float m = -INFINITY;
#pragma unroll
        for (int kb = 0; kb < NKB; ++kb)
#pragma unroll
            for (int r = 0; r < 16; ++r) {
                const int key = kb * 32 + (r & 3) + 8 * (r >> 2) + 4 * kh;
                float v = s[kb][r] * 0.125f;
                if (key >= L || (causal && key > query)) v = -INFINITY;
                s[kb][r] = v;
                m = fmaxf(m, v);
            }
        m = fmaxf(m, __shfl_xor(m, 32));
        float z = 0.f;
#pragma unroll
        for (int kb = 0; kb < NKB; ++kb)
#pragma unroll
            for (int r = 0; r < 16; ++r) {
                const float e2 = __expf(s[kb][r] - m);
                s[kb][r] = e2;
                z += e2;
            }
        z += __shfl_xor(z, 32);
        inv = 1.f / z;
    }
    __syncthreads();
    if (!qwave) return;
    f16x o[2], ol[2];
#pragma unroll
    for (int db = 0; db < 2; ++db)
#pragma unroll
        for (int r = 0; r < 16; ++r) { o[db][r] = 0.f; ol[db][r] = 0.f; }
#pragma unroll
    for (int ks = 0; ks < 2 * NKB; ++ks) {
        h8 ph, pl;
#pragma unroll
        for (int e = 0; e < 8; ++e) {
            const float pv = s[ks >> 1][(2 * (ks & 1) + (e >> 2)) * 4 + (e & 3)] * inv;
            ph[e] = (half_t)pv;
            pl[e] = (half_t)((pv - (float)ph[e]) * 2048.f);
        }
#pragma unroll
        for (int db = 0; db < 2; ++db) {
            const h8 vf = *(const h8*)(vt + (db * 32 + lr) * VROW + (ks * 16 + kh * 8) * 2);
            o[db] = mfma32(vf, ph, o[db]);
            ol[db] = mfma32(vf, pl, ol[db]);
        }
    }
    if (pair < n_pairs && query < L) {
        half_t* op = out + ((long long)img * L + query) * D + h * 64 + 4 * kh;
#pragma unroll
        for (int db = 0; db < 2; ++db)
#pragma unroll
            for (int g = 0; g < 4; ++g) {
                h4 w;
#pragma unroll
                for (int q = 0; q < 4; ++q) w[q] = (half_t)(o[db][g * 4 + q] + ol[db][g * 4 + q] * (1.f / 2048.f));
                *(h4*)(op + db * 32 + 8 * g) = w;
            }
    }
}

// ... 6 lines not shown
    const int pair = blockIdx.x / nqb, qblk = blockIdx.x - pair * nqb;
    const int img = pair / heads, h = pair - img * heads, D = heads * 64;
    const half_t* base = qkv + (long long)img * L * 3 * D + h * 64;
    const long long ts = 3LL * D;
    const int q0 = qblk * 128 + wave * 32, query = q0 + lr;
    int nkt = (L + 63) / 64;
    if (causal) nkt = min(nkt, (min(qblk * 128 + 127, L - 1) >> 6) + 1);
    const int wkt = q0 >= L ? 0 : causal ? min(nkt, ((q0 + 31) >> 6) + 1) : nkt;
    const int sk = t >> 3, sd8 = t & 7, vtok = 2 * (t & 31), vd8 = t >> 5;
    const int vr_ = vtok & 31, vg = vr_ >> 3;
    const int vpos = ((vtok >> 5) * 2 + (vg >> 1)) * 16 + ((vr_ >> 2) & 1) * 8 + (vg & 1) * 4 + (vr_ & 3);
    h8 kr[2], vr[2];
    auto stage_load = [&](int kt) {
        const int k0 = kt * 64;
#pragma unroll
        for (int u = 0; u < 2; ++u) {
            kr[u] = *(const h8*)(base + (long long)min(k0 + sk + 32 * u, L - 1) * ts + D + sd8 * 8);
            vr[u] = *(const h8*)(base + (long long)min(k0 + vtok + u, L - 1) * ts + 2 * D + vd8 * 8);
        }
    };
    auto stage_write = [&](int kt, int buf) {
        const int k0 = kt * 64;
#pragma unroll
        for (int u = 0; u < 2; ++u) *(h8*)(kls[buf] + (sk + 32 * u) * ROW + sd8 * 16) = kr[u];
        const bool ok0 = k0 + vtok < L, ok1 = k0 + vtok + 1 < L;
#pragma unroll
        for (int j = 0; j < 8; ++j) {
            h2 w;
            w[0] = ok0 ? vr[0][j] : (half_t)0.f;
            w[1] = ok1 ? vr[1][j] : (half_t)0.f;
            *(h2*)(vls[buf] + (vd8 * 8 + j) * ROW + vpos * 2) = w;
        }
    };
    h8 qf[4];
    {
        const half_t* qp = base + (long long)min(query, L - 1) * ts + kh * 8;
#pragma unroll
        for (int kk = 0; kk < 4; ++kk) qf[kk] = *(const h8*)(qp + kk * 16);
    }
    f16x o[2], ol[2];
#pragma unroll
    for (int db = 0; db < 2; ++db)
#pragma unroll
        for (int r = 0; r < 16; ++r) { o[db][r] = 0.f; ol[db][r] = 0.f; }
    float m = -INFINITY, z = 0.f;
    stage_load(0);
    stage_write(0, 0);
    __syncthreads();
    for (int kt = 0; kt < nkt; ++kt) {
        const int buf = kt & 1;
        const bool work = kt < wkt;
        f16x s[2];
        if (work) {
            const char* kl = kls[buf];
#pragma unroll
            for (int kb = 0; kb < 2; ++kb) {
#pragma unroll
                for (int r = 0; r < 16; ++r) s[kb][r] = 0.f;
#pragma unroll
                for (int kk = 0; kk < 4; ++kk) {
                    const h8 kf = *(const h8*)(kl + (kb * 32 + lr) * ROW + (kk * 16 + kh * 8) * 2);
                    s[kb] = mfma32(kf, qf[kk], s[kb]);
                }
            }
        }
        if (kt + 1 < nkt) stage_load(kt + 1);
        if (work) {
            const int k0 = kt * 64;
            float mt = -INFINITY;
#pragma unroll
            for (int kb = 0; kb < 2; ++kb)
#pragma unroll
                for (int r = 0; r < 16; ++r) {
                    const int key = k0 + kb * 32 + (r & 3) + 8 * (r >> 2) + 4 * kh;
                    float v = s[kb][r] * 0.125f;
                    if (key >= L || (causal && key > query)) v = -INFINITY;
                    s[kb][r] = v;
                    mt = fmaxf(mt, v);
                }
            mt = fmaxf(mt, __shfl_xor(mt, 32));
            const float mn = fmaxf(m, mt);
            const float alpha = __expf(m - mn);
            m = mn;
            float zt = 0.f;
#pragma unroll
            for (int kb = 0; kb < 2; ++kb)
#pragma unroll
                for (int r = 0; r < 16; ++r) {
                    const float e2 = __expf(s[kb][r] - mn);
                    s[kb][r] = e2;
                    zt += e2;
                }
            z = z * alpha + zt;
            if (__any(alpha != 1.f)) {
#pragma unroll
                for (int db = 0; db < 2; ++db)
#pragma unroll
                    for (int r = 0; r < 16; ++r) { o[db][r] *= alpha; ol[db][r] *= alpha; }
            }
            const char* vl = vls[buf];
#pragma unroll
            for (int ks = 0; ks < 4; ++ks) {
                h8 ph, pl;
#pragma unroll
                for (int e = 0; e < 8; ++e) {
                    const float pv = s[ks >> 1][(2 * (ks & 1) + (e >> 2)) * 4 + (e & 3)];
                    ph[e] = (half_t)pv;
                    pl[e] = (half_t)((pv - (float)ph[e]) * 2048.f);
                }
#pragma unroll
                for (int db = 0; db < 2; ++db) {
                    const h8 vf = *(const h8*)(vl + (db * 32 + lr) * ROW + (ks * 16 + kh * 8) * 2);
                    o[db] = mfma32(vf, ph, o[db]);
                    ol[db] = mfma32(vf, pl, ol[db]);
                }
            }
        }
        if (kt + 1 < nkt) stage_write(kt + 1, buf ^ 1);
        __syncthreads();
    }
    if (query < L) {
        z += __shfl_xor(z, 32);
        const float inv = 1.f / z;
        half_t* op = out + ((long long)img * L + query) * D + h * 64 + 4 * kh;
#pragma unroll
        for (int db = 0; db < 2; ++db)
#pragma unroll
            for (int g = 0; g < 4; ++g) {
                h4 w;
#pragma unroll
                for (int q = 0; q < 4; ++q) w[q] = (half_t)((o[db][g * 4 + q] + ol[db][g * 4 + q] * (1.f / 2048.f)) * inv);
                *(h4*)(op + db * 32 + 8 * g) = w;
            }
    }
}

void launch_attention(const half_t* qkv, int n_img, int L, int heads, int hd, int causal, half_t* out,
                      hipStream_t st) {
    (void)hd;
    if (L <= 64) {
        const int n_pairs = n_img * heads;
        hipLaunchKernelGGL(attention_mfma_kernel<2>, dim3((n_pairs + 1) / 2), dim3(256), 0, st, qkv, L, heads, n_pairs, causal, out);
        return;
    }
    if (L <= 96) {
        const int n_pairs = n_img * heads;
        hipLaunchKernelGGL(attention_mfma_kernel<3>, dim3(n_pairs), dim3(256), 0, st, qkv, L, heads, n_pairs, causal, out);
        return;
    }
    const int nqb = (L + 127) / 128;
    hipLaunchKernelGGL(attention_stream_kernel, dim3((unsigned)((long long)n_img * heads * nqb)), dim3(256), 0, st, qkv, L, heads, causal, out);
}

__global__ void cosine_kernel(const float* feat, const float* target, int D, float* sim) {
    const int p = blockIdx.x, lane = threadIdx.x;
    float xy = 0.f, xx = 0.f, yy = 0.f;
    for (int i = lane; i < D; i += 64) {
        const float a = feat[(long long)p * D + i], b = target[i];
        xy += a * b; xx += a * a; yy += b * b;
    }
    xy = wsum(xy); xx = wsum(xx); yy = wsum(yy);
    if (lane == 0) sim[p] = xy / fmaxf(sqrtf(xx) * sqrtf(yy), 1e-8f);
}
void launch_cosine(const float* feat, const float* target, int P, int D, float* sim, hipStream_t st) {
    hipLaunchKernelGGL(cosine_kernel, dim3(P), dim3(64), 0, st, feat, target, D, sim);
}

__global__ void assemble_F_kernel(const float* sim, const float* dis, int P, int n_obj, float* F) {
    const int p = blockIdx.x * blockDim.x + threadIdx.x;
    if (p >= P) return;
    F[(long long)p * n_obj] = -sim[p];
    if (n_obj == 2) F[(long long)p * n_obj + 1] = fmaxf(1.f - dis[p], 0.f);
}
void launch_assemble_F(const float* sim, const float* dis, int P, int n_obj, float* F, hipStream_t st) {
    hipLaunchKernelGGL(assemble_F_kernel, dim3((P + 63) / 64), dim3(64), 0, st, sim, dis, P, n_obj, F);
}

__global__ void image_patches_kernel(const float* img, int n, int S, int ps, int ld, half_t* patches) {
    const int G = S / ps;
    const long long idx = (long long)blockIdx.x * blockDim.x + threadIdx.x;
    if (idx >= (long long)n * 3 * S * S) return;
    const int X = (int)(idx % S), Y = (int)((idx / S) % S);
    const int c = (int)((idx / ((long long)S * S)) % 3), b = (int)(idx / ((long long)S * S * 3));
    const int gy = Y / ps, iy = Y - gy * ps, gx = X / ps, ix = X - gx * ps;
    const long long row = ((long long)b * G + gy) * G + gx;
    patches[row * ld + ((long long)c * ps + iy) * ps + ix] = (half_t)img[idx];
}
void launch_image_patches(const float* img, int n, int S, int ps, int ld, half_t* patches, hipStream_t st) {
    const long long total = (long long)n * 3 * S * S;
    hipLaunchKernelGGL(image_patches_kernel, dim3((unsigned)((total + 255) / 256)), dim3(256), 0, st, img, n, S, ps, ld, patches);
}
```

### clip_glass_amd/csrc/ops.hip

```cpp
#include <string.h>

#include <string>
#include <vector>

#include "../../include/glass_ops.h"
#include "engine.h"
#include "kernels.h"

namespace {
struct Dev {
    std::vector<void*> ptrs;
    ~Dev() {
        for (void* p : ptrs) hipFree(p);
    }
    template <typename T>
    T* alloc(size_t n) {
        void* q = nullptr;
        if (hipMalloc(&q, (n ? n : 1) * sizeof(T)) != hipSuccess) return nullptr;
        ptrs.push_back(q);
        return (T*)q;
    }
    half_t* up16(const float* src, size_t n) {
        if (!src) return nullptr;
        std::vector<_Float16> h(n);
// ... 14 lines not shown
        return d;
    }
};
int down16(float* dst, const half_t* src, size_t n) {
    std::vector<_Float16> h(n);
    GLASS_HIP(hipMemcpy(h.data(), src, n * sizeof(half_t), hipMemcpyDeviceToHost));
    for (size_t i = 0; i < n; ++i) dst[i] = (float)h[i];
    return GLASS_OK;
}
int finish() {
    GLASS_HIP(hipDeviceSynchronize());
    GLASS_HIP(hipGetLastError());
    return GLASS_OK;
}
}

#define OPREQ(cond, msg)               \
    do {                               \
        if (!(cond)) {                 \
            glass_set_error(msg);      \
            return GLASS_ERR_ARG;      \
        }                              \
    } while (0)

extern "C" int glass_op_conv(int32_t device, const glass_conv_desc* d) {
    OPREQ(d && d->x && d->w && d->y, "null argument");
    OPREQ(d->Cin % 16 == 0, "Cin must be a multiple of 16");
    OPREQ(d->out_scale > 0.f, "out_scale must be positive (the epilogues fold it into the activation constants: max(v k1, v k2))");
    GLASS_HIP(hipSetDevice(device));
    Dev dv;
    ConvParams p;
    memset(&p, 0, sizeof p);
    const size_t xin = (size_t)(d->broadcast_x ? 1 : d->B) * d->H * d->W * d->Cin;
    p.x = dv.up16(d->x, xin);
    p.x_bstride = d->broadcast_x ? 0 : (long long)d->H * d->W * d->Cin;
    p.B = d->B; p.H = d->H; p.W = d->W; p.Cin = d->Cin;
    p.KS = d->KS; p.stride = d->stride; p.pad = d->pad; p.up = d->up;
    p.Cout = d->Cout; p.Neff = d->up ? 4 * d->Cout : d->Cout;
    p.Ho = d->Ho; p.Wo = d->Wo;
    p.Hc = d->up ? d->H : d->Ho; p.Wc = d->up ? d->W : d->Wo;
    std::vector<_Float16> pk;
    if (d->up) {
        OPREQ(d->KS == 3 && d->stride == 1 && d->pad == 1 && d->Ho == 2 * d->H, "up conv expects KS 3 / pad 1");
        glass_fold_upconv(d->w, d->Cout, d->Cin, pk);
    } else {
        glass_pack_conv(d->w, d->Cout, d->Cin, d->KS, d->Cin, pk);
    }
    p.w = dv.up16v(pk);
    if (d->up) {
        std::vector<_Float16> pk2;
        glass_pack_conv(d->w, d->Cout, d->Cin, 3, d->Cin, pk2);
        p.w_up = dv.up16v(pk2);
    }
    p.sn = dv.up32(d->sn, (size_t)d->B * d->Cin); p.sn_stride = d->Cin;
    p.sn16 = dv.up16(d->sn, (size_t)d->B * d->Cin);
    p.dscale = dv.up32(d->dscale, (size_t)d->B * d->Cout); p.ds_stride = d->Cout;
    p.batch_size = d->batch_size > 0 ? d->batch_size : 1;
    p.noise = dv.up32(d->noise, (size_t)(d->B / p.batch_size) * d->Ho * d->Wo);
    p.noise_strength = d->noise_strength;
    p.bias = dv.up32(d->bias, d->Cout);
    p.act = d->act;
    const size_t nout = (size_t)d->B * d->Ho * d->Wo * d->Cout;
    p.res = dv.up16(d->res, nout);
    p.out_scale = d->out_scale;
    half_t* y = dv.alloc<half_t>(nout);
    p.y = y;
    OPREQ(p.x && p.w && y, "device allocation failed");
    if (d->skip_x) {
        OPREQ(d->skip_w && (d->impl == 2 || d->impl == 5), "fused skip branch: impl 2 / 5 with skip_x and skip_w");
        std::vector<_Float16> pks;
        glass_pack_conv(d->skip_w, d->Cout, d->Cin, 1, d->Cin, pks);
        p.skip_w = dv.up16v(pks);
        p.skip_x = dv.up16(d->skip_x, (size_t)d->B * d->Ho * d->Wo * d->Cin);
    }
    half_t* xs_dev = nullptr;
    const size_t nxs = (size_t)d->B * (d->H / 2) * (d->W / 2) * d->Cin;
    if (d->xs_out) {
        OPREQ(d->impl == 2 || d->impl == 5, "blur-down by-product: impl 2 / 5");
        xs_dev = dv.alloc<half_t>(nxs);
        p.xs_out = xs_dev;
    }
    float* yrgb = nullptr;
    const size_t nrgb = (size_t)d->B * 3 * d->Ho * d->Wo;
    if (d->trgb_yout) {
        OPREQ((d->impl == 4 || d->impl == 2 || d->impl == 5) && d->trgb_w && d->trgb_b && d->trgb_sn && d->trgb_smax,
              "fused toRGB: impl 2 / 4 / 5 and all of w / b / sn / smax");
        p.trgb_w = dv.up32(d->trgb_w, 3 * (size_t)d->Cout); p.trgb_b = dv.up32(d->trgb_b, 3);
        p.trgb_sn = dv.up32(d->trgb_sn, (size_t)d->B * d->Cout); p.trgb_sn_stride = d->Cout;
        p.trgb_smax = dv.up32(d->trgb_smax, d->B); p.trgb_smax_stride = 1;
        p.trgb_yprev = dv.up32(d->trgb_yprev, (size_t)d->B * 3 * (d->Ho / 2) * (d->Wo / 2));
        yrgb = dv.alloc<float>(nrgb);
        p.trgb_yout = yrgb;
        if (d->impl == 4) {
            p.y = nullptr;
        } else {
            half_t* tab = dv.alloc<half_t>((size_t)d->B * 32 * d->Cout);
            launch_trgb_tables(p.trgb_w, p.trgb_sn, p.trgb_sn_stride, p.trgb_smax, p.trgb_smax_stride, d->B, d->Cout, tab, 0);
            p.trgb_tab = tab;
        }
    }
    p.x_planar8 = d->x_planar8;
    p.x_planar32 = d->x_planar32;
    if (d->impl == 1) { if (!launch_conv_direct(p, 0)) { glass_set_error("direct conv: unsupported launch"); return GLASS_ERR_ARG; } }
    else if (d->impl == 3) {
        if (!launch_upconv_fused(p, 0)) { glass_set_error("fused up-conv: unsupported shape"); return GLASS_ERR_ARG; }
    } else if (d->impl == 2) {
        if (!launch_conv_tiled(p, 0)) { glass_set_error("tiled conv: unsupported shape"); return GLASS_ERR_ARG; }
    } else if (d->impl == 4) {
        if (!launch_conv_stream(p, 0)) { glass_set_error("streaming conv: unsupported shape"); return GLASS_ERR_ARG; }
    } else if (d->impl == 6) {
        const long long cap_a = (long long)p.Hc * p.Wc * p.KS * p.KS * p.Cin, cap_c = (long long)p.Hc * p.Wc * p.Neff;
        half_t* wa = dv.alloc<half_t>((size_t)(cap_a * p.B));
        float* wc = dv.alloc<float>((size_t)(cap_c * p.B));
        if (!launch_conv_gemm(p, wa, cap_a, wc, cap_c, 0)) { glass_set_error("im2col + GEMM conv: unsupported shape"); return GLASS_ERR_ARG; }
    } else if (d->impl == 5) {
        if (p.skip_x) {
            if (!launch_conv_s2(p, 0, true)) { glass_set_error("LDS-DMA stride-2 conv: unsupported shape"); return GLASS_ERR_ARG; }
        } else if (!launch_conv_glds(p, 0)) { glass_set_error("LDS-DMA conv: unsupported shape"); return GLASS_ERR_ARG; }
    } else if (!(d->up && launch_upconv_fused(p, 0)) && !launch_conv_stream(p, 0) && !launch_conv_tiled(p, 0) && !launch_conv_direct(p, 0)) {
        glass_set_error("no kernel accepts this convolution");
        return GLASS_ERR_ARG;
    }
    int rc = finish();
    if (rc) return rc;
    if (yrgb) {
        GLASS_HIP(hipMemcpy(d->trgb_yout, yrgb, nrgb * sizeof(float), hipMemcpyDeviceToHost));
        return p.y ? down16(d->y, y, nout) : GLASS_OK;
    }
    if (xs_dev && (rc = down16(d->xs_out, xs_dev, nxs))) return rc;
    return down16(d->y, y, nout);
}

extern "C" int glass_op_gemm(int32_t device, int32_t M, int32_t N, int32_t K, const float* a, const float* w,
                             const float* bias, int32_t mode, int32_t impl, float* out) {
    OPREQ(a && w && out && K % 16 == 0, "bad argument");
    GLASS_HIP(hipSetDevice(device));
    Dev dv;
    GemmParams g;
    memset(&g, 0, sizeof g);
    g.a = dv.up16(a, (size_t)M * K); g.w = dv.up16(w, (size_t)N * K); g.M = M; g.N = N; g.K = K;
    g.bias = dv.up32(bias, N); g.mode = mode; g.ldo = N;
    const size_t n = (size_t)M * N;
    half_t* o16 = nullptr; float* o32 = nullptr;
    if (mode <= 1) { o16 = dv.alloc<half_t>(n); g.out16 = o16; }
    else { o32 = mode == 2 ? dv.up32(out, n) : dv.alloc<float>(n); g.out32 = o32; }
    if (impl == 1) launch_gemm_direct(g, 0);
    else if (impl == 2) {
        if (!launch_gemm_tiled(g, 0)) { glass_set_error("tiled gemm: unsupported shape"); return GLASS_ERR_ARG; }
    } else if (!launch_gemm_tiled(g, 0)) launch_gemm_direct(g, 0);
    int rc = finish();
    if (rc) return rc;
    if (o16) return down16(out, o16, n);
    GLASS_HIP(hipMemcpy(out, o32, n * sizeof(float), hipMemcpyDeviceToHost));
    return GLASS_OK;
}

extern "C" int glass_op_dense(int32_t device, int32_t P, int32_t K, int32_t N, const float* x, const float* wt,
                              const float* bias, int32_t in_sq, int32_t mode, const float* eps_row, float* out) {
    OPREQ(x && wt && out, "null argument");
    GLASS_HIP(hipSetDevice(device));
    Dev dv;
    float* dx = dv.up32(x, (size_t)P * K); float* dw = dv.up32(wt, (size_t)K * N); float* db = dv.up32(bias, N);
    float* de = dv.up32(eps_row, P); float* dout = dv.alloc<float>((size_t)P * N);
    launch_dense(dx, K, P, K, dw, N, db, dout, N, in_sq, mode, de, 1, 0);
    int rc = finish();
    if (rc) return rc;
    GLASS_HIP(hipMemcpy(out, dout, (size_t)P * N * sizeof(float), hipMemcpyDeviceToHost));
    return GLASS_OK;
}

extern "C" int glass_op_torgb(int32_t device, int32_t B, int32_t H, int32_t C, const float* x, const float* wrgb,
                              const float* bias, const float* sn, const float* smax, const float* yprev, float* yout) {
    OPREQ(x && wrgb && bias && sn && smax && yout, "null argument");
    GLASS_HIP(hipSetDevice(device));
    Dev dv;
    half_t* dx = dv.up16(x, (size_t)B * H * H * C);
    float* dw = dv.up32(wrgb, 3 * C); float* db = dv.up32(bias, 3); float* ds = dv.up32(sn, (size_t)B * C);
    float* dm = dv.up32(smax, B); float* dp = dv.up32(yprev, (size_t)B * 3 * (H / 2) * (H / 2));
    float* dy = dv.alloc<float>((size_t)B * 3 * H * H);
    OPREQ(launch_torgb(dx, B, H, H, C, dw, db, ds, C, dm, 1, dp, dy, 0), "toRGB: channel width not instantiated");
    int rc = finish();
    if (rc) return rc;
    GLASS_HIP(hipMemcpy(yout, dy, (size_t)B * 3 * H * H * sizeof(float), hipMemcpyDeviceToHost));
    return GLASS_OK;
}

extern "C" int glass_op_blur(int32_t device, int32_t mode, int32_t B, int32_t H, int32_t C, const float* x, float* out) {
    OPREQ(x && out && C % 8 == 0, "bad argument");
    GLASS_HIP(hipSetDevice(device));
    Dev dv;
    half_t* dx = dv.up16(x, (size_t)B * H * H * C);
    OPREQ(mode != 2 || blur_pad2_planar32_ok(C), "blur in 32-channel planes: C must be 32 x a power of two, <= 512");
    const int Ho = mode != 1 ? H + 1 : H / 2;
    half_t* dy = dv.alloc<half_t>((size_t)B * Ho * Ho * C);
    if (mode != 1) launch_blur_pad2(dx, B, H, H, C, dy, 0, mode == 2);
    else launch_blur_down(dx, B, H, H, C, dy, 0);
    int rc = finish();
    if (rc) return rc;
    return down16(out, dy, (size_t)B * Ho * Ho * C);
}

extern "C" int glass_op_dblock_down(int32_t device, int32_t B, int32_t R, int32_t Cin, int32_t Cout, const float* h,
                                    const float* x, const float* w1, const float* wskip, const float* b1, float* y) {
    OPREQ(h && x && w1 && wskip && b1 && y, "bad argument");
    GLASS_HIP(hipSetDevice(device));
    Dev dv;
    half_t* dh = dv.up16(h, (size_t)B * R * R * Cin);
    half_t* dx = dv.up16(x, (size_t)B * R * R * Cin);
    std::vector<_Float16> pk;
    glass_pack_conv(w1, Cout, Cin, 3, Cin, pk);
    half_t* dw1 = dv.up16v(pk);
    glass_pack_conv(wskip, Cout, Cin, 1, Cin, pk);
    half_t* dws = dv.up16v(pk);
    float* db = dv.up32(b1, Cout);
    const int Ro = R / 2;
    half_t* dxs = dv.alloc<half_t>((size_t)B * Ro * Ro * Cin);
    half_t* dy = dv.alloc<half_t>((size_t)B * Ro * Ro * Cout);
    OPREQ(conv_down_supported(R, Cin, Cout), "conv_down: unsupported shape");
    launch_blur_down(dx, B, R, R, Cin, dxs, 0);
    OPREQ(launch_conv_down(dh, dxs, dw1, dws, db, dy, B, R, Cin, Cout, 0) != nullptr, "conv_down: unsupported shape");
    int rc = finish();
    if (rc) return rc;
    return down16(y, dy, (size_t)B * Ro * Ro * Cout);
}

extern "C" int glass_op_dblock0(int32_t device, int32_t B, int32_t R, int32_t impl, const float* y, const float* frgb_w, const float* frgb_b,
                                const float* w0, const float* b0, const float* w1, const float* wskip, const float* b1, float* out) {
    OPREQ(y && frgb_w && frgb_b && w0 && b0 && w1 && wskip && b1 && out && B > 0 && R > 0, "bad argument");
    GLASS_HIP(hipSetDevice(device));
    Dev dv;
    const int Cin = 32, Cout = 64, Ro = R / 2;
    float* dy = dv.up32(y, (size_t)B * 3 * R * R);
    float* dfw = dv.up32(frgb_w, Cin * 3); float* dfb = dv.up32(frgb_b, Cin);
    std::vector<_Float16> pk;
    glass_pack_conv(w0, Cin, Cin, 3, Cin, pk);
    half_t* dw0 = dv.up16v(pk);
    glass_pack_conv(w1, Cout, Cin, 3, Cin, pk);
    half_t* dw1 = dv.up16v(pk);
    glass_pack_conv(wskip, Cout, Cin, 1, Cin, pk);
    half_t* dws = dv.up16v(pk);
    float* db0 = dv.up32(b0, Cin); float* db1 = dv.up32(b1, Cout);
    half_t* dout = dv.alloc<half_t>((size_t)B * Ro * Ro * Cout);
    OPREQ(dy && dw0 && dw1 && dws && dout, "device allocation failed");
    if (impl == 0 || impl == 2) {
        OPREQ(launch_dblock0(dy, dfw, dfb, dw0, db0, dw1, dws, db1, dout, B, R, Cin, Cout, 0, impl == 2) != nullptr, "dblock0: unsupported shape");
    } else {
        half_t* dh = dv.alloc<half_t>((size_t)B * R * R * Cin);
        half_t* dxs = dv.alloc<half_t>((size_t)B * Ro * Ro * Cin);
        OPREQ(dh && dxs, "device allocation failed");
        ConvParams p = conv_defaults();
        p.x = dh; p.x_bstride = (long long)R * R * Cin; p.B = B; p.H = p.W = R; p.Cin = Cin; p.Hc = p.Wc = R; p.KS = 3; p.pad = 1;
        p.w = dw0; p.Cout = p.Neff = Cin; p.Ho = p.Wo = R; p.bias = db0; p.act = 1; p.y = dh;
        p.rgb_y = dy; p.rgb_w = dfw; p.rgb_b = dfb; p.rgb_xs_out = dxs;
        OPREQ(launch_conv_stream(p, 0) != nullptr, "dblock0 (two-kernel form): conv_stream<fromrgb> does not take this shape");
        OPREQ(launch_conv_down(dh, dxs, dw1, dws, db1, dout, B, R, Cin, Cout, 0) != nullptr, "dblock0 (two-kernel form): conv_down does not take this shape");
    }
    int rc = finish();
    if (rc) return rc;
    return down16(out, dout, (size_t)B * Ro * Ro * Cout);
}

extern "C" int glass_op_fromrgb(int32_t device, int32_t B, int32_t R, int32_t Cout, const float* y, const float* w,
                                const float* bias, float* out) {
    OPREQ(y && w && bias && out && Cout % 8 == 0, "bad argument");
    GLASS_HIP(hipSetDevice(device));
    Dev dv;
    float* dy = dv.up32(y, (size_t)B * 3 * R * R); float* dw = dv.up32(w, Cout * 3); float* db = dv.up32(bias, Cout);
    half_t* dout = dv.alloc<half_t>((size_t)B * R * R * Cout);
    launch_fromrgb(dy, B, R, Cout, dw, db, dout, 0);
    int rc = finish();
    if (rc) return rc;
    return down16(out, dout, (size_t)B * R * R * Cout);
}

extern "C" int glass_op_mbstd(int32_t device, int32_t B, int32_t hw, int32_t C, int32_t Cpad, int32_t batch_size,
                              int32_t group, const float* x, float* out) {
    OPREQ(x && out && B % batch_size == 0 && batch_size % group == 0 && group <= 8, "bad argument");
    GLASS_HIP(hipSetDevice(device));
    Dev dv;
    half_t* dx = dv.up16(x, (size_t)B * hw * C);
    half_t* dy = dv.alloc<half_t>((size_t)B * hw * Cpad);
    launch_mbstd(dx, B, hw, C, Cpad, batch_size, group, 1e-8f, dy, 0);
    int rc = finish();
    if (rc) return rc;
    return down16(out, dy, (size_t)B * hw * Cpad);
}

extern "C" int glass_op_resize(int32_t device, int32_t B, int32_t R, int32_t S, int32_t ps, const float* y, float* patches) {
    OPREQ(y && patches && S % ps == 0, "bad argument");
    GLASS_HIP(hipSetDevice(device));
    Dev dv;
    float* dy = dv.up32(y, (size_t)B * 3 * R * R);
    const size_t n = (size_t)B * 3 * S * S;
    half_t* dp = dv.alloc<half_t>(n);
    launch_resize_patches(dy, B, R, S, ps, 3 * ps * ps, dp, 0);
    int rc = finish();
    if (rc) return rc;
    return down16(patches, dp, n);
}

extern "C" int glass_op_layernorm(int32_t device, int32_t M, int32_t D, const float* x, const float* g, const float* b, float* out) {
    OPREQ(x && g && b && out, "null argument");
    GLASS_HIP(hipSetDevice(device));
    Dev dv;
    float* dx = dv.up32(x, (size_t)M * D); float* dg = dv.up32(g, D); float* db = dv.up32(b, D);
    float* dout = dv.alloc<float>((size_t)M * D);
// ... 271 lines not shown
```

### clip_glass_amd/ops.py

```python
import ctypes as C

import numpy as np

from .engine import _check, _f32, _fp, load_library


class ConvDesc(C.Structure):
    _fields_ = [("B", C.c_int32), ("H", C.c_int32), ("W", C.c_int32), ("Cin", C.c_int32), ("Cout", C.c_int32),
                ("KS", C.c_int32), ("stride", C.c_int32), ("pad", C.c_int32), ("up", C.c_int32),
                ("Ho", C.c_int32), ("Wo", C.c_int32), ("broadcast_x", C.c_int32), ("act", C.c_int32),
                ("batch_size", C.c_int32), ("impl", C.c_int32),
                ("noise_strength", C.c_float), ("out_scale", C.c_float),
                ("x", C.POINTER(C.c_float)), ("w", C.POINTER(C.c_float)), ("sn", C.POINTER(C.c_float)),
                ("dscale", C.POINTER(C.c_float)), ("noise", C.POINTER(C.c_float)), ("bias", C.POINTER(C.c_float)),
                ("res", C.POINTER(C.c_float)), ("y", C.POINTER(C.c_float)),
                ("trgb_w", C.POINTER(C.c_float)), ("trgb_b", C.POINTER(C.c_float)), ("trgb_sn", C.POINTER(C.c_float)),
                ("trgb_smax", C.POINTER(C.c_float)), ("trgb_yprev", C.POINTER(C.c_float)),
                ("trgb_yout", C.POINTER(C.c_float)),
                ("skip_x", C.POINTER(C.c_float)), ("skip_w", C.POINTER(C.c_float)), ("xs_out", C.POINTER(C.c_float)),
                ("x_planar8", C.c_int32), ("x_planar32", C.c_int32)]


def to_planar8(a):
    B, H, W, Cc = a.shape
    return np.ascontiguousarray(a.reshape(B, H, W, Cc // 8, 8).transpose(0, 3, 1, 2, 4))


def to_planar32(a):
    B, H, W, Cc = a.shape
    return np.ascontiguousarray(a.reshape(B, H, W, Cc // 32, 32).transpose(0, 3, 1, 2, 4))


def from_planar32(a, B, H, W, Cc):
    return np.ascontiguousarray(a.reshape(B, Cc // 32, H, W, 32).transpose(0, 2, 3, 1, 4)).reshape(B, H, W, Cc)


def from_planar8(a, B, H, W, Cc):
    return np.ascontiguousarray(a.reshape(B, Cc // 8, H, W, 8).transpose(0, 2, 3, 1, 4)).reshape(B, H, W, Cc)


def _opt(a):
    if a is None:
        return None, None
    a = _f32(a)
    return a, _fp(a)


def conv(x, w, *, stride=1, pad=None, up=False, sn=None, dscale=None, noise=None, noise_strength=0.0,
         batch_size=1, bias=None, act=False, res=None, out_scale=1.0, impl=0, broadcast_x=False, B=None, device=0,
         torgb=None, skip=None, xs_out=None, planar_x=False, both=False, planar32_x=False):
    lib = load_library()
    x = _f32(x); w = _f32(w)
    Bx, H, W, Cin = x.shape
    if planar_x:
        x = to_planar8(x)
    if planar32_x:
        x = to_planar32(x)
    B = B if B is not None else Bx
    Cout, _, KS, _ = w.shape
    pad = (KS // 2) if pad is None else pad
    if up:
        Ho, Wo = 2 * H, 2 * W
    else:
        Ho, Wo = (H + 2 * pad - KS) // stride + 1, (W + 2 * pad - KS) // stride + 1
    y = np.empty((B, Ho, Wo, Cout), dtype=np.float32)
    d = ConvDesc()
    d.B, d.H, d.W, d.Cin, d.Cout = B, H, W, Cin, Cout
    d.KS, d.stride, d.pad, d.up, d.Ho, d.Wo = KS, stride, pad, int(up), Ho, Wo
    d.broadcast_x, d.act, d.batch_size, d.impl = int(broadcast_x), int(act), batch_size, impl
    d.noise_strength, d.out_scale = noise_strength, out_scale
    d.x_planar8 = int(planar_x)
    d.x_planar32 = int(planar32_x)
    keep = []
    d.x, d.w, d.y = _fp(x), _fp(w), _fp(y)
    for name, val in (("sn", sn), ("dscale", dscale), ("noise", noise), ("bias", bias), ("res", res)):
        a, p = _opt(val)
        keep.append(a)
        if p is not None:
            setattr(d, name, p)
    if skip is not None:
        for name, val in zip(("skip_x", "skip_w"), skip):
            a, p = _opt(val)
            keep.append(a)
            setattr(d, name, p)
    if xs_out is not None:
        d.xs_out = _fp(xs_out)
    yrgb = None
    if torgb is not None:
        yrgb = np.empty((B, 3, Ho, Wo), dtype=np.float32)
        for name in ("w", "b", "sn", "smax", "yprev"):
            a, p = _opt(torgb.get(name))
            keep.append(a)
            if p is not None:
                setattr(d, "trgb_" + name, p)
        d.trgb_yout = _fp(yrgb)
    lib.glass_op_conv.argtypes = [C.c_int32, C.POINTER(ConvDesc)]
    _check(lib, lib.glass_op_conv(device, C.byref(d)))
    if both:
        return yrgb, y
    return yrgb if yrgb is not None else y


def gemm(a, w, bias=None, mode=3, impl=0, acc=None, device=0):
    lib = load_library()
    a = _f32(a); w = _f32(w)
    M, K = a.shape
    N = w.shape[0]
    out = _f32(acc).copy() if acc is not None else np.empty((M, N), dtype=np.float32)
    b, bp = _opt(bias)
    lib.glass_op_gemm.argtypes = [C.c_int32] * 4 + [C.POINTER(C.c_float)] * 3 + [C.c_int32, C.c_int32, C.POINTER(C.c_float)]
    _check(lib, lib.glass_op_gemm(device, M, N, K, _fp(a), _fp(w), bp, mode, impl, _fp(out)))
    return out


def dense(x, wt, bias=None, in_sq=False, mode=0, eps_row=None, device=0):
    lib = load_library()
    x = _f32(x); wt = _f32(wt)
    P, K = x.shape
    N = wt.shape[1]
    out = np.empty((P, N), dtype=np.float32)
    b, bp = _opt(bias)
    e, ep = _opt(eps_row)
    fp = C.POINTER(C.c_float)
    lib.glass_op_dense.argtypes = [C.c_int32] * 4 + [fp, fp, fp, C.c_int32, C.c_int32, fp, fp]
    _check(lib, lib.glass_op_dense(device, P, K, N, _fp(x), _fp(wt), bp, int(in_sq), mode, ep, _fp(out)))
    return out


def torgb(x, wrgb, bias, sn, smax, yprev=None, device=0):
    lib = load_library()
    x = _f32(x)
    B, H, _, Cc = x.shape
    wrgb, bias, sn, smax = _f32(wrgb), _f32(bias), _f32(sn), _f32(smax)
    yp, ypp = _opt(yprev)
    out = np.empty((B, 3, H, H), dtype=np.float32)
    fp = C.POINTER(C.c_float)
    lib.glass_op_torgb.argtypes = [C.c_int32] * 4 + [fp] * 7
    _check(lib, lib.glass_op_torgb(device, B, H, Cc, _fp(x), _fp(wrgb), _fp(bias), _fp(sn), _fp(smax), ypp, _fp(out)))
    return out


def blur(x, mode, device=0):
    lib = load_library()
    x = _f32(x)
    B, H, _, Cc = x.shape
    Ho = H + 1 if mode != 1 else H // 2
    out = np.empty((B, Ho, Ho, Cc), dtype=np.float32)
    fp = C.POINTER(C.c_float)
    lib.glass_op_blur.argtypes = [C.c_int32] * 5 + [fp, fp]
    _check(lib, lib.glass_op_blur(device, mode, B, H, Cc, _fp(x), _fp(out)))
    return from_planar32(out, B, Ho, Ho, Cc) if mode == 2 else out


def dblock_down(h, x, w1, wskip, b1, device=0):
    lib = load_library()
    h, x, w1, wskip, b1 = _f32(h), _f32(x), _f32(w1), _f32(wskip), _f32(b1)
    B, R, _, Cin = h.shape
    Cout = w1.shape[0]
    out = np.empty((B, R // 2, R // 2, Cout), dtype=np.float32)
    fp = C.POINTER(C.c_float)
    lib.glass_op_dblock_down.argtypes = [C.c_int32] * 5 + [fp] * 6
    _check(lib, lib.glass_op_dblock_down(device, B, R, Cin, Cout, _fp(h), _fp(x), _fp(w1), _fp(wskip), _fp(b1), _fp(out)))
    return out


def dblock0(y, frgb_w, frgb_b, w0, b0, w1, wskip, b1, impl=0, device=0):
    lib = load_library()
    y, frgb_w, frgb_b, w0, b0, w1, wskip, b1 = (_f32(a) for a in (y, frgb_w, frgb_b, w0, b0, w1, wskip, b1))
    B, _, R, _ = y.shape
    out = np.empty((B, R // 2, R // 2, 64), dtype=np.float32)
    fp = C.POINTER(C.c_float)
    lib.glass_op_dblock0.argtypes = [C.c_int32] * 4 + [fp] * 9
    _check(lib, lib.glass_op_dblock0(device, B, R, impl, _fp(y), _fp(frgb_w), _fp(frgb_b), _fp(w0), _fp(b0), _fp(w1), _fp(wskip),
                                     _fp(b1), _fp(out)))
    return from_planar8(out, B, R // 2, R // 2, 64) if impl == 2 else out


def fromrgb(y, w, bias, device=0):
    lib = load_library()
    y, w, bias = _f32(y), _f32(w), _f32(bias)
    B, _, R, _ = y.shape
    Cout = w.shape[0]
    out = np.empty((B, R, R, Cout), dtype=np.float32)
    fp = C.POINTER(C.c_float)
    lib.glass_op_fromrgb.argtypes = [C.c_int32] * 4 + [fp] * 4
    _check(lib, lib.glass_op_fromrgb(device, B, R, Cout, _fp(y), _fp(w), _fp(bias), _fp(out)))
    return out


def mbstd(x, Cpad, batch_size, group=4, device=0):
    lib = load_library()
    x = _f32(x)
    B, hw, Cc = x.shape
    out = np.empty((B, hw, Cpad), dtype=np.float32)
    fp = C.POINTER(C.c_float)
    lib.glass_op_mbstd.argtypes = [C.c_int32] * 7 + [fp, fp]
    _check(lib, lib.glass_op_mbstd(device, B, hw, Cc, Cpad, batch_size, group, _fp(x), _fp(out)))
    return out


def resize(y, S, ps, device=0):
    lib = load_library()
    y = _f32(y)
    B, _, R, _ = y.shape
    G = S // ps
    out = np.empty((B * G * G, 3 * ps * ps), dtype=np.float32)
    fp = C.POINTER(C.c_float)
    lib.glass_op_resize.argtypes = [C.c_int32] * 5 + [fp, fp]
    _check(lib, lib.glass_op_resize(device, B, R, S, ps, _fp(y), _fp(out)))
    return out


def layernorm(x, g, b, device=0):
    lib = load_library()
    x, g, b = _f32(x), _f32(g), _f32(b)
    out = np.empty_like(x)
    fp = C.POINTER(C.c_float)
    lib.glass_op_layernorm.argtypes = [C.c_int32] * 3 + [fp] * 4
    _check(lib, lib.glass_op_layernorm(device, x.shape[0], x.shape[1], _fp(x), _fp(g), _fp(b), _fp(out)))
    return out


def attention(qkv, n_img, L, heads, causal=False, device=0):
    lib = load_library()
    qkv = _f32(qkv)
    out = np.empty((n_img * L, heads * 64), dtype=np.float32)
    fp = C.POINTER(C.c_float)
    lib.glass_op_attention.argtypes = [C.c_int32] * 5 + [fp, fp]
    _check(lib, lib.glass_op_attention(device, n_img, L, heads, int(causal), _fp(qkv), _fp(out)))
    return out


def noise(n_mb, hw, layer, mb0, generation, seed, device=0):
    lib = load_library()
    out = np.empty((n_mb, hw), dtype=np.float32)
    lib.glass_op_noise.argtypes = [C.c_int32, C.c_int32, C.c_int32, C.c_uint32, C.c_uint32, C.c_uint32, C.c_uint64,
                                   C.POINTER(C.c_float)]
    _check(lib, lib.glass_op_noise(device, n_mb, hw, layer, mb0, generation, seed, _fp(out)))
    return out


def gpt2_sample(logits, temperature, top_k, seed, generation, first_row, step, purpose=0, device=0):
    lib = load_library()
    lg = _f32(logits)
    rows, V = lg.shape
    out = np.empty(rows, dtype=np.int32)
    ip = C.POINTER(C.c_int32)
    lib.glass_op_gpt2_sample.argtypes = [C.c_int32, C.c_int32, C.c_int32, C.POINTER(C.c_float), C.c_float, C.c_int32, C.c_uint64,
                                         C.c_int32, C.c_int32, C.c_int32, C.c_int32, ip]
    _check(lib, lib.glass_op_gpt2_sample(device, rows, V, _fp(lg), float(temperature), int(top_k), int(seed) & 0xFFFFFFFFFFFFFFFF,
                                         int(generation), int(first_row), int(step), int(purpose), out.ctypes.data_as(ip)))
    return out


GPT2_GEMM_FORMS = {"prefill": 0, "decode": 1, "step": 2, "rowblk": 3}


def gpt2_gemm(a, w, bias=None, mode=0, form="step", res=None, ln=None, pst_in=None, want_pst=False, width=None, device=0):
    lib = load_library()
    a = np.asarray(a, dtype=np.float32)
    assert a.ndim == 2 and a.strides[1] == 4 and a.strides[0] % 4 == 0
    M, K = a.shape
    lda = a.strides[0] // 4 if M > 1 else K
    abuf = np.zeros((M, lda), dtype=np.float32)
    abuf[:, :K] = a
    if lda > K:
        abuf[:, K:] = np.nan
# ... 104 lines not shown
```

### include/glass_ops.h

```cpp
#ifndef GLASS_OPS_H
#define GLASS_OPS_H
#include <stdint.h>
#ifdef __cplusplus
extern "C" {
#endif

typedef struct glass_conv_desc {
    int32_t B, H, W, Cin, Cout;
    int32_t KS, stride, pad;
    int32_t up;
    int32_t Ho, Wo;
    int32_t broadcast_x;
    int32_t act;
    int32_t batch_size;
    int32_t impl;
    float noise_strength, out_scale;
    const float* x;
    const float* w;
    const float* sn;
    const float* dscale;
    const float* noise;
    const float* bias;
    const float* res;
    float* y;
    const float* trgb_w;
    const float* trgb_b;
    const float* trgb_sn;
    const float* trgb_smax;
    const float* trgb_yprev;
    float* trgb_yout;
    const float* skip_x;
    const float* skip_w;
    float* xs_out;
    int32_t x_planar8;
    int32_t x_planar32;
} glass_conv_desc;

int glass_op_conv(int32_t device, const glass_conv_desc* d);
int glass_op_gemm(int32_t device, int32_t M, int32_t N, int32_t K, const float* a, const float* w,
                  const float* bias, int32_t mode, int32_t impl, float* out);
int glass_op_dense(int32_t device, int32_t P, int32_t K, int32_t N, const float* x, const float* wt ,
                   const float* bias, int32_t in_sq, int32_t mode, const float* eps_row, float* out);
int glass_op_torgb(int32_t device, int32_t B, int32_t H, int32_t C, const float* x, const float* wrgb ,
                   const float* bias, const float* sn, const float* smax, const float* yprev, float* yout);
int glass_op_blur(int32_t device, int32_t mode , int32_t B, int32_t H, int32_t C,
                  const float* x, float* out);
int glass_op_dblock_down(int32_t device, int32_t B, int32_t R, int32_t Cin, int32_t Cout, const float* h, const float* x,
                         const float* w1, const float* wskip, const float* b1, float* y);
int glass_op_dblock0(int32_t device, int32_t B, int32_t R, int32_t impl, const float* y, const float* frgb_w, const float* frgb_b,
                     const float* w0, const float* b0, const float* w1, const float* wskip, const float* b1, float* out);
int glass_op_fromrgb(int32_t device, int32_t B, int32_t R, int32_t Cout, const float* y ,
                     const float* w , const float* bias, float* out );
int glass_op_mbstd(int32_t device, int32_t B, int32_t hw, int32_t C, int32_t Cpad, int32_t batch_size, int32_t group,
                   const float* x, float* out);
int glass_op_resize(int32_t device, int32_t B, int32_t R, int32_t S, int32_t ps, const float* y ,
                    float* patches );
int glass_op_layernorm(int32_t device, int32_t M, int32_t D, const float* x, const float* g, const float* b, float* out);
int glass_op_attention(int32_t device, int32_t n_img, int32_t L, int32_t heads, int32_t causal, const float* qkv,
                       float* out);
int glass_op_noise(int32_t device, int32_t n_mb, int32_t hw, uint32_t layer, uint32_t mb0, uint32_t generation,
                   uint64_t seed, float* out);
int glass_op_gpt2_sample(int32_t device, int32_t rows, int32_t V, const float* logits, float temperature, int32_t top_k,
                         uint64_t seed, int32_t generation, int32_t first_row, int32_t step, int32_t purpose, int32_t* out);
int glass_op_gpt2_gemm(int32_t device, int32_t form, int32_t M, int32_t N, int32_t K, int32_t lda, int32_t mode, int32_t width,
                       const float* a, const float* w, const float* bias, const float* lng, const float* lnb, const float* pst_in,
                       int32_t np_in, float* out, float* stats_out, float* pst_out, int32_t* splits);
int glass_op_gpt2_attention(int32_t device, int32_t form, int32_t P, int32_t nd, int32_t past, int32_t Tmax, int32_t heads, int32_t S,
                            const float* qkv, const float* bias, float* kc, float* vc, float* out);
int glass_op_gpt2_head(int32_t device, int32_t M, int32_t V, int32_t K, int32_t tail, const float* x, const float* wte, const float* lng,
                       const float* lnb, const float* wpe, int32_t npos, int32_t past, int32_t step, float* logits, float* pair_val,
                       int32_t* pair_idx, int32_t* token, float* stats, float* x_next, float* stats_next, int32_t* state);
int glass_op_gpt2_embed_step(int32_t device, int32_t M, int32_t V, int32_t K, const int32_t* token, const float* wte, const float* wpe,
                             int32_t npos, int32_t past, int32_t step, float* x, float* stats);
int glass_op_mfma_probe(int32_t device, const float* a , const float* b , float* d );

int glass_host_pack_conv(const float* w, int32_t Cout, int32_t Cin, int32_t KS, int32_t up, float* out);

#ifdef __cplusplus
}
#endif
#endif
```

Before: 2283 candidates/s.

## Fuse CLIP layernorms into GEMM loaders via epilogue-computed block statistics

The residual-writing GEMM epilogues (attn_out, mlp_proj) now emit per-32-column mean and M2 partial statistics. The following QKV and MLP-fc GEMMs combine these partials into per-row mean and rstd and normalise the fp32 residual on the fly in the A-tile loader. This removes the standalone layernorm kernels and the fp16 normalised intermediate buffer from the CLIP tower, and the head's layernorm, projection and cosine steps become a single kernel. In exchange the A operand is read as fp32, which doubles its load traffic, and the loader carries extra registers, which may reduce occupancy.

```diff
diff --git a/clip_glass_amd/csrc/common.h b/clip_glass_amd/csrc/common.h
--- a/clip_glass_amd/csrc/common.h
+++ b/clip_glass_amd/csrc/common.h
@@ -194,4 +194,36 @@
     int g_on, g_h, g_w, g_hc, g_wc, g_stride, g_pad, g_ks, g_cin;
     long long g_xbs;
     int ld;
+    const float* a32;
+    const float* ln_g;
+    const float* ln_b;
+    const float* ln_stats;
+    float* ln_stats_out;
 };
+
+#define LN_BLK 32
+#define LN_MAX_W 1024
+__device__ __forceinline__ float ln_apply(float x, float mean, float rstd, float g, float b) {
+    return __builtin_fmaf((x - mean) * rstd, g, b);
+}
+__device__ __forceinline__ void ln_chan(float& mean, float& m2, int nb, float bm, float bm2) {
+    const float na = (float)(nb * LN_BLK), n = na + (float)LN_BLK;
+    const float d = bm - mean;
+    mean = __builtin_fmaf(d, (float)LN_BLK / n, mean);
+    m2 = __builtin_fmaf(d * d, na * (float)LN_BLK / n, m2 + bm2);
+}
+__device__ __forceinline__ void ln_combine(const float* st, int nblk, float& mean, float& rstd) {
+    f4 v[LN_MAX_W / LN_BLK / 2];
+#pragma unroll
+    for (int b = 0; b < LN_MAX_W / LN_BLK / 2; ++b) v[b] = 2 * b < nblk ? *(const f4*)(st + 4 * b) : f4{0.f, 0.f, 0.f, 0.f};
+    float m = v[0][0], m2 = v[0][1];
+    ln_chan(m, m2, 1, v[0][2], v[0][3]);
+#pragma unroll
+    for (int b = 1; b < LN_MAX_W / LN_BLK / 2; ++b)
+        if (2 * b < nblk) {
+            ln_chan(m, m2, 2 * b, v[b][0], v[b][1]);
+            ln_chan(m, m2, 2 * b + 1, v[b][2], v[b][3]);
+        }
+    mean = m;
+    rstd = rsqrtf(m2 / (float)(nblk * LN_BLK) + 1e-5f);
+}
diff --git a/clip_glass_amd/csrc/engine.cpp b/clip_glass_amd/csrc/engine.cpp
--- a/clip_glass_amd/csrc/engine.cpp
+++ b/clip_glass_amd/csrc/engine.cpp
@@ -630,6 +630,7 @@
     if ((rc = dev_alloc(e, &e->d_pe, (size_t)P * G * G * W))) return rc;
     if ((rc = dev_alloc(e, &e->d_x, (size_t)P * T * W))) return rc;
     if ((rc = dev_alloc(e, &e->d_ln16, (size_t)P * T * W))) return rc;
+    if ((rc = dev_alloc(e, &e->d_lnstats, (size_t)P * T * (W / LN_BLK + 1) * 2))) return rc;
     if ((rc = dev_alloc(e, &e->d_qkv, (size_t)P * T * 3 * W))) return rc;
     if ((rc = dev_alloc(e, &e->d_attn, (size_t)P * T * W))) return rc;
     if ((rc = dev_alloc(e, &e->d_hid, (size_t)P * T * 4 * W))) return rc;
@@ -1224,50 +1225,66 @@
     }
     run_clip(e, P, l0, 1 << 20);
 }
+static bool clip_tower_fused(int M, int W) { return M >= 64 && W % 64 == 0 && W <= LN_MAX_W; }
 void run_clip(glass_engine* e, int P, int l0, int l1) {
     const glass_config& c = e->cfg;
     const int W = c.clip_width, ps = c.clip_patch, G = c.clip_res / ps, T = G * G + 1, M = P * T;
+    const bool fused = clip_tower_fused(M, W);
+    float* stats = fused ? e->d_lnstats : nullptr;
     GemmParams g;
     if (l0 == 0) {
         memset(&g, 0, sizeof g);
         g.a = e->d_patches; g.w = e->c_patch_w; g.M = P * G * G; g.N = W; g.K = clip_patch_k(c); g.mode = 3; g.out32 = e->d_pe; g.ldo = W; g.cand_rows = G * G;
         run_gemm(e, g, "clip.patch_embed");
         Prof pr(e, "clip.embed_lnpre", 0, 8.0 * M * W);
-        launch_embed_lnpre(e->d_pe, e->c_cls, e->c_pos, e->c_lnpre_g, e->c_lnpre_b, P, T, W, e->d_x, e->cur);
-    }
+        launch_embed_lnpre(e->d_pe, e->c_cls, e->c_pos, e->c_lnpre_g, e->c_lnpre_b, P, T, W, e->d_x, stats, e->cur);
+    }
+    auto ln_gemm = [&](const float* lg, const float* lb, const half_t* w, const float* bias, int N, int mode, half_t* out, const char* tag) {
+        memset(&g, 0, sizeof g);
+        g.w = w; g.M = M; g.N = N; g.K = W; g.bias = bias; g.mode = mode; g.out16 = out; g.ldo = N; g.cand_rows = T;
+        if (!fused) {
+            {
+                Prof pr(e, "clip.layernorm", 0, 6.0 * M * W);
+                launch_layernorm(e->d_x, W, M, W, lg, lb, e->d_ln16, nullptr, e->cur);
+            }
+            g.a = e->d_ln16;
+            run_gemm(e, g, tag);
+            return;
+        }
+        g.a32 = e->d_x; g.ln_g = lg; g.ln_b = lb; g.ln_stats = stats;
+        Prof pr(e, tag, 2.0 * M * N * W, 4.0 * M * W + 8.0 * M * (W / LN_BLK) + 2.0 * ((double)N * W + (double)M * N));
+        const char* k = launch_gemm_tiled(g, e->cur);
+        if (!k) {
+            if (e->launch_error.empty()) e->launch_error = std::string("gemm_tiled refused the normalising loader of ") + tag;
+            k = "(refused)";
+        }
+        if (pr.on) pr.pe.name = std::string(tag) + "@" + k;
+        if (e->profiling) e->tag_kernel[tag] = k;
+    };
     for (int li = l0 < 0 ? 0 : l0; li < l1 && li < (int)e->cblk.size(); ++li) {
         auto& b = e->cblk[li];
-        {
-            Prof pr(e, "clip.layernorm", 0, 6.0 * M * W);
-            launch_layernorm(e->d_x, W, M, W, b.ln1_g, b.ln1_b, e->d_ln16, nullptr, e->cur);
-        }
-        memset(&g, 0, sizeof g);
-        g.a = e->d_ln16; g.w = b.w_qkv; g.M = M; g.N = 3 * W; g.K = W; g.bias = b.b_qkv; g.mode = 0; g.out16 = e->d_qkv; g.ldo = 3 * W; g.cand_rows = T;
-        run_gemm(e, g, "clip.qkv");
+        ln_gemm(b.ln1_g, b.ln1_b, b.w_qkv, b.b_qkv, 3 * W, 0, e->d_qkv, "clip.qkv");
         {
             Prof pr(e, "clip.attention", 4.0 * P * c.clip_heads * (double)T * T * 64, 8.0 * M * W);
             launch_attention(e->d_qkv, P, T, c.clip_heads, 64, 0, e->d_attn, e->cur);
         }
         memset(&g, 0, sizeof g);
-        g.a = e->d_attn; g.w = b.w_out; g.M = M; g.N = W; g.K = W; g.bias = b.b_out; g.mode = 2; g.out32 = e->d_x; g.ldo = W; g.cand_rows = T;
+        g.a = e->d_attn; g.w = b.w_out; g.M = M; g.N = W; g.K = W; g.bias = b.b_out; g.mode = 2; g.out32 = e->d_x; g.ldo = W; g.cand_rows = T; g.ln_stats_out = stats;
         run_gemm(e, g, "clip.attn_out");
-        {
-            Prof pr(e, "clip.layernorm", 0, 6.0 * M * W);
-            launch_layernorm(e->d_x, W, M, W, b.ln2_g, b.ln2_b, e->d_ln16, nullptr, e->cur);
-        }
+        ln_gemm(b.ln2_g, b.ln2_b, b.w_fc, b.b_fc, 4 * W, 1, e->d_hid, "clip.mlp_fc");
         memset(&g, 0, sizeof g);
-        g.a = e->d_ln16; g.w = b.w_fc; g.M = M; g.N = 4 * W; g.K = W; g.bias = b.b_fc; g.mode = 1; g.out16 = e->d_hid; g.ldo = 4 * W; g.cand_rows = T;
-        run_gemm(e, g, "clip.mlp_fc");
-        memset(&g, 0, sizeof g);
-        g.a = e->d_hid; g.w = b.w_proj; g.M = M; g.N = W; g.K = 4 * W; g.bias = b.b_proj; g.mode = 2; g.out32 = e->d_x; g.ldo = W; g.cand_rows = T;
+        g.a = e->d_hid; g.w = b.w_proj; g.M = M; g.N = W; g.K = 4 * W; g.bias = b.b_proj; g.mode = 2; g.out32 = e->d_x; g.ldo = W; g.cand_rows = T; g.ln_stats_out = stats;
         run_gemm(e, g, "clip.mlp_proj");
     }
     if (l1 >= (int)e->cblk.size()) {
         Prof pr(e, "clip.head", 2.0 * P * W * c.clip_embed, 4.0 * W * c.clip_embed);
-        launch_layernorm(e->d_x, (long long)T * W, P, W, e->c_lnpost_g, e->c_lnpost_b, nullptr, e->d_cls, e->cur);
-        launch_dense(e->d_cls, W, P, W, e->c_proj, c.clip_embed, nullptr, e->d_feat, c.clip_embed, 0, 0, nullptr, 0,
-                     e->cur);
-        launch_cosine(e->d_feat, e->d_target, P, c.clip_embed, e->d_sim, e->cur);
+        if (!fused || !launch_clip_head(e->d_x, (long long)T * W, P, W, e->c_lnpost_g, e->c_lnpost_b, e->c_proj, c.clip_embed, e->d_target, e->d_feat,
+                                        e->d_sim, e->cur)) {
+            launch_layernorm(e->d_x, (long long)T * W, P, W, e->c_lnpost_g, e->c_lnpost_b, nullptr, e->d_cls, e->cur);
+            launch_dense(e->d_cls, W, P, W, e->c_proj, c.clip_embed, nullptr, e->d_feat, c.clip_embed, 0, 0, nullptr, 0,
+                         e->cur);
+            launch_cosine(e->d_feat, e->d_target, P, c.clip_embed, e->d_sim, e->cur);
+        }
     }
 }
 
diff --git a/clip_glass_amd/csrc/engine.h b/clip_glass_amd/csrc/engine.h
--- a/clip_glass_amd/csrc/engine.h
+++ b/clip_glass_amd/csrc/engine.h
@@ -170,6 +170,7 @@
     half_t *d_patches = nullptr, *d_ln16 = nullptr, *d_qkv = nullptr, *d_attn = nullptr, *d_hid = nullptr;
     float *d_pe = nullptr, *d_x = nullptr, *d_cls = nullptr, *d_feat = nullptr, *d_sim = nullptr, *d_dis = nullptr,
           *d_F = nullptr, *d_dh = nullptr, *d_dh_part = nullptr;
+    float* d_lnstats = nullptr;
     half_t* d_dfin = nullptr;
     float* h_pinned = nullptr;
     size_t h_pinned_bytes = 0;
@@ -265,7 +266,9 @@
 void run_gemm(glass_engine* e, const GemmParams& p, const char* tag);
 ConvParams conv_defaults();
 void run_clip(glass_engine* e, int P, int l0, int l1);
+#ifndef GLASS_CLIP_SERIAL_LAYERS
 #define GLASS_CLIP_SERIAL_LAYERS 1
+#endif
 std::vector<_Float16> to_half(const float* p, size_t n, float scale = 1.f);
 std::vector<float> scaled(const float* p, size_t n, float scale);
 std::vector<float> transposed(const float* W, int N, int K, float coef);
diff --git a/clip_glass_amd/csrc/gemm_tiled.hip b/clip_glass_amd/csrc/gemm_tiled.hip
--- a/clip_glass_amd/csrc/gemm_tiled.hip
+++ b/clip_glass_amd/csrc/gemm_tiled.hip
@@ -4,7 +4,7 @@
 
 #define GROWB 144
 
-template <int BN, bool GATHER = false>
+template <int BN, bool GATHER = false, bool LNA = false>
 __global__ __launch_bounds__(256, 2) void gemm_tiled_kernel(GemmParams p) {
     if (p.batch > 1) {
         p.a += (long long)blockIdx.z * p.a_bs;
@@ -29,6 +29,8 @@
     const int part = t & 7;
 
     h8 ra[NA], rb[NB];
+    f4 rx[NA][2], rg[2], rbt[2];
+    float lmean[NA], lrstd[NA];
     long long gbase[GATHER ? NA : 1];
     int giy[GATHER ? NA : 1], gix[GATHER ? NA : 1], okm = 0;
     if (GATHER) {
@@ -53,6 +55,18 @@
                 ra[k] = *(const h8*)(p.a + (ok ? gbase[k] + toff : (long long)part * 8));
                 okm |= (ok ? 1 : 0) << k;
             }
+        } else if (LNA) {
+#pragma unroll
+            for (int k = 0; k < NA; ++k) {
+                const float* xr = p.a32 + (long long)min(m0 + (t >> 3) + 32 * k, p.M - 1) * p.K + k0 + part * 8;
+                rx[k][0] = *(const f4*)xr;
+                rx[k][1] = *(const f4*)(xr + 4);
+            }
+#pragma unroll
+            for (int h = 0; h < 2; ++h) {
+                rg[h] = *(const f4*)(p.ln_g + k0 + part * 8 + 4 * h);
+                rbt[h] = *(const f4*)(p.ln_b + k0 + part * 8 + 4 * h);
+            }
         } else {
 #pragma unroll
         for (int k = 0; k < NA; ++k) {
@@ -70,8 +84,18 @@
     };
     auto store = [&]() {
         const h8 zero = {0, 0, 0, 0, 0, 0, 0, 0};
+        if (LNA) {
+#pragma unroll
+            for (int k = 0; k < NA; ++k) {
+                h8 v;
+#pragma unroll
+                for (int e = 0; e < 8; ++e) v[e] = (half_t)ln_apply(rx[k][e >> 2][e & 3], lmean[k], lrstd[k], rg[e >> 2][e & 3], rbt[e >> 2][e & 3]);
+                *(h8*)(As + ((t >> 3) + 32 * k) * GROWB + part * 16) = v;
+            }
+        } else {
 #pragma unroll
         for (int k = 0; k < NA; ++k) *(h8*)(As + ((t >> 3) + 32 * k) * GROWB + part * 16) = (!GATHER || ((okm >> k) & 1)) ? ra[k] : zero;
+        }
 #pragma unroll
         for (int k = 0; k < NB; ++k) *(h8*)(Bs + ((t >> 3) + 32 * k) * GROWB + part * 16) = rb[k];
     };
@@ -85,6 +109,13 @@
             for (int q = 0; q < 16; ++q) acc[i][j][q] = 0.f;
 
     load(0);
+    if (LNA) {
+        __shared__ float lnst[128][2];
+        if (t < 128) ln_combine(p.ln_stats + (long long)min(m0 + t, p.M - 1) * (p.K / LN_BLK) * 2, p.K / LN_BLK, lnst[t][0], lnst[t][1]);
+        __syncthreads();
+#pragma unroll
+        for (int k = 0; k < NA; ++k) { lmean[k] = lnst[(t >> 3) + 32 * k][0]; lrstd[k] = lnst[(t >> 3) + 32 * k][1]; }
+    }
     for (int k0 = 0; k0 < p.K; k0 += 64) {
         if (k0 > 0) __syncthreads();
         store();
@@ -128,6 +159,7 @@
         if (m >= p.M) continue;
 #pragma unroll
         for (int j = 0; j < NJ; ++j) {
+            f4 ob[4];
 #pragma unroll
             for (int g = 0; g < 4; ++g) {
                 const int n = n0 + wn * (BN / 2) + j * 32 + 8 * g + 4 * kh;
@@ -151,6 +183,27 @@
                         for (int q = 0; q < 4; ++q) o[q] = p.mode == 4 ? lrelu_sqrt2(v[q]) : v[q];
                     }
                     *(f4*)(p.out32 + oi) = o;
+                    ob[g] = o;
+                }
+            }
+            if (p.mode == 2 && p.ln_stats_out) {
+                float s = 0.f;
+#pragma unroll
+                for (int g = 0; g < 4; ++g)
+#pragma unroll
+                    for (int q = 0; q < 4; ++q) s += ob[g][q];
+                s += __shfl_xor(s, 32);
+                const float bm = s * (1.f / 32.f);
+                float q2 = 0.f;
+#pragma unroll
+                for (int g = 0; g < 4; ++g)
+#pragma unroll
+                    for (int q = 0; q < 4; ++q) { const float d = ob[g][q] - bm; q2 = __builtin_fmaf(d, d, q2); }
+                q2 += __shfl_xor(q2, 32);
+                if (kh == 0) {
+                    float* sp = p.ln_stats_out + ((long long)m * (p.N / LN_BLK) + (n0 + wn * (BN / 2) + j * 32) / LN_BLK) * 2;
+                    sp[0] = bm;
+                    sp[1] = q2;
                 }
             }
         }
@@ -164,6 +217,19 @@
     const long long gz_n = p.cand_batch ? GLASS_NOMINAL_POP : gz;
     const bool fills = gx_n * (p.N / 128) * gz_n >= 256;
     if (p.g_on && (!p.kpt || p.kpt != p.g_cin || p.g_cin % 64 != 0)) return nullptr;
+    if (p.ln_stats_out && (p.mode != 2 || p.ldo != p.N || gz > 1)) return nullptr;
+    if (p.a32) {
+        if (p.g_on || p.batch > 1 || p.kpt || p.ld || p.K > LN_MAX_W || !p.ln_g || !p.ln_b || !p.ln_stats) return nullptr;
+        if (p.N % 128 == 0 && fills) {
+            hipLaunchKernelGGL((gemm_tiled_kernel<128, false, true>), dim3(8 * ((gx * (p.N / 128) + 7) / 8)), dim3(256), 0, st, p);
+            return "gemm_tiled_kernel<128,false,true>";
+        }
+        if (p.N % 64 == 0) {
+            hipLaunchKernelGGL((gemm_tiled_kernel<64, false, true>), dim3(8 * ((gx * (p.N / 64) + 7) / 8)), dim3(256), 0, st, p);
+            return "gemm_tiled_kernel<64,false,true>";
+        }
+        return nullptr;
+    }
     if (p.N % 128 == 0 && fills) {
         if (p.g_on) {
             hipLaunchKernelGGL((gemm_tiled_kernel<128, true>), dim3(8 * ((gx * (p.N / 128) + 7) / 8), 1, gz), dim3(256), 0, st, p);
@@ -182,3 +248,12 @@
     }
     return nullptr;
 }
+
+__global__ void ln_stats_combine_kernel(const float* st, int M, int W, float* mean, float* rstd) {
+    const int m = blockIdx.x * blockDim.x + threadIdx.x;
+    if (m >= M) return;
+    ln_combine(st + (long long)m * (W / LN_BLK) * 2, W / LN_BLK, mean[m], rstd[m]);
+}
+void launch_ln_stats_combine(const float* st, int M, int W, float* mean, float* rstd, hipStream_t s) {
+    hipLaunchKernelGGL(ln_stats_combine_kernel, dim3((M + 63) / 64), dim3(64), 0, s, st, M, W, mean, rstd);
+}
diff --git a/clip_glass_amd/csrc/kernels.h b/clip_glass_amd/csrc/kernels.h
--- a/clip_glass_amd/csrc/kernels.h
+++ b/clip_glass_amd/csrc/kernels.h
@@ -60,7 +60,11 @@
                   half_t* out, hipStream_t st);
 
 void launch_embed_lnpre(const float* patch_emb, const float* cls, const float* pos, const float* g,
-                        const float* b, int P, int T, int D, float* x, hipStream_t st);
+                        const float* b, int P, int T, int D, float* x, float* stats, hipStream_t st);
+void launch_row_stats(const float* x, int M, int D, float* stats, hipStream_t st);
+void launch_ln_stats_combine(const float* stats, int M, int W, float* mean, float* rstd, hipStream_t st);
+bool launch_clip_head(const float* x, long long row_stride, int P, int W, const float* g, const float* b, const float* proj, int E,
+                      const float* target, float* feat, float* sim, hipStream_t st);
 void launch_embed_text(const int* tokens, const float* tok_emb, const float* pos, int n_rows, int ctx, int D, float* x,
                        hipStream_t st);
 void launch_layernorm(const float* x, long long row_stride, int M, int D, const float* g, const float* b,
diff --git a/clip_glass_amd/csrc/kernels_clip.hip b/clip_glass_amd/csrc/kernels_clip.hip
--- a/clip_glass_amd/csrc/kernels_clip.hip
+++ b/clip_glass_amd/csrc/kernels_clip.hip
@@ -8,8 +8,28 @@
     return v;
 }
 
+__device__ __forceinline__ void row_block_stats(const float (&v)[16], int D, float* st) {
+    const int lane = threadIdx.x & 63;
+#pragma unroll
+    for (int k = 0; k < 16; ++k) {
+        if (64 * k < D) {
+            float s = v[k];
+#pragma unroll
+            for (int o = 16; o > 0; o >>= 1) s += __shfl_xor(s, o);
+            const float bm = s * (1.f / 32.f), d = v[k] - bm;
+            float q = d * d;
+#pragma unroll
+            for (int o = 16; o > 0; o >>= 1) q += __shfl_xor(q, o);
+            if ((lane & 31) == 0) {
+                st[(2 * k + (lane >> 5)) * 2] = bm;
+                st[(2 * k + (lane >> 5)) * 2 + 1] = q;
+            }
+        }
+    }
+}
+
 template <typename LoadF>
-__device__ __forceinline__ void ln_row(LoadF load, int D, const float* g, const float* b, half_t* o16, float* o32) {
+__device__ __forceinline__ void ln_row(LoadF load, int D, const float* g, const float* b, half_t* o16, float* o32, float* st = nullptr) {
     const int lane = threadIdx.x & 63;
     if (D <= 1024) {
         float v[16];
@@ -27,11 +47,13 @@
         for (int k = 0; k < 16; ++k) {
             const int i = lane + 64 * k;
             if (i < D) {
-                const float o = (v[k] - mean) * rstd * g[i] + b[i];
+                const float o = ln_apply(v[k], mean, rstd, g[i], b[i]);
                 if (o16) o16[i] = (half_t)o;
                 if (o32) o32[i] = o;
-            }
-        }
+                v[k] = o;
+            }
+        }
+        if (st) row_block_stats(v, D, st);
         return;
     }
     float s = 0.f;
@@ -41,7 +63,7 @@
     for (int i = lane; i < D; i += 64) { const float d = load(i) - mean; q += d * d; }
     const float rstd = rsqrtf(wsum(q) / (float)D + 1e-5f);
     for (int i = lane; i < D; i += 64) {
-        const float v = (load(i) - mean) * rstd * g[i] + b[i];
+        const float v = ln_apply(load(i), mean, rstd, g[i], b[i]);
         if (o16) o16[i] = (half_t)v;
         if (o32) o32[i] = v;
     }
@@ -49,18 +71,31 @@
 
 __global__ __launch_bounds__(256) void embed_lnpre_kernel(const float* pe, const float* cls, const float* pos,
                                                           const float* g, const float* b, int P, int T, int D,
-                                                          float* x) {
+                                                          float* x, float* stats) {
     const int row = blockIdx.x * 4 + (threadIdx.x >> 6);
     if (row >= P * T) return;
     const int p = row / T, t = row - p * T;
     const float* src = t == 0 ? cls : pe + ((long long)p * (T - 1) + (t - 1)) * D;
     const float* ps = pos + (long long)t * D;
-    ln_row([&](int i) { return src[i] + ps[i]; }, D, g, b, nullptr, x + (long long)row * D);
+    ln_row([&](int i) { return src[i] + ps[i]; }, D, g, b, nullptr, x + (long long)row * D,
+           stats ? stats + (long long)row * (D / LN_BLK) * 2 : nullptr);
 }
 void launch_embed_lnpre(const float* patch_emb, const float* cls, const float* pos, const float* g,
-                        const float* b, int P, int T, int D, float* x, hipStream_t st) {
+                        const float* b, int P, int T, int D, float* x, float* stats, hipStream_t st) {
     hipLaunchKernelGGL(embed_lnpre_kernel, dim3((P * T + 3) / 4), dim3(256), 0, st, patch_emb, cls, pos, g, b, P,
-                       T, D, x);
+                       T, D, x, stats);
+}
+
+__global__ __launch_bounds__(256) void row_stats_kernel(const float* x, int M, int D, float* stats) {
+    const int row = blockIdx.x * 4 + (threadIdx.x >> 6), lane = threadIdx.x & 63;
+    if (row >= M) return;
+    float v[16];
+#pragma unroll
+    for (int k = 0; k < 16; ++k) v[k] = lane + 64 * k < D ? x[(long long)row * D + lane + 64 * k] : 0.f;
+    row_block_stats(v, D, stats + (long long)row * (D / LN_BLK) * 2);
+}
+void launch_row_stats(const float* x, int M, int D, float* stats, hipStream_t st) {
+    hipLaunchKernelGGL(row_stats_kernel, dim3((M + 3) / 4), dim3(256), 0, st, x, M, D, stats);
 }
 
 __global__ void embed_text_kernel(const int* tokens, const float* tok_emb, const float* pos, int ctx, int D, float* x) {
@@ -373,15 +408,52 @@
     hipLaunchKernelGGL(attention_stream_kernel, dim3((unsigned)((long long)n_img * heads * nqb)), dim3(256), 0, st, qkv, L, heads, causal, out);
 }
 
-__global__ void cosine_kernel(const float* feat, const float* target, int D, float* sim) {
-    const int p = blockIdx.x, lane = threadIdx.x;
+__device__ __forceinline__ void cosine_row(const float* f, const float* target, int D, float* sim) {
+    const int lane = threadIdx.x & 63;
     float xy = 0.f, xx = 0.f, yy = 0.f;
     for (int i = lane; i < D; i += 64) {
-        const float a = feat[(long long)p * D + i], b = target[i];
-        xy += a * b; xx += a * a; yy += b * b;
+        const float a = f[i], b = target[i];
+        xy = __builtin_fmaf(a, b, xy); xx = __builtin_fmaf(a, a, xx); yy = __builtin_fmaf(b, b, yy);
     }
     xy = wsum(xy); xx = wsum(xx); yy = wsum(yy);
-    if (lane == 0) sim[p] = xy / fmaxf(sqrtf(xx) * sqrtf(yy), 1e-8f);
+    if (lane == 0) *sim = xy / fmaxf(sqrtf(xx) * sqrtf(yy), 1e-8f);
+}
+__global__ void cosine_kernel(const float* feat, const float* target, int D, float* sim) {
+    cosine_row(feat + (long long)blockIdx.x * D, target, D, sim + blockIdx.x);
+}
+
+#define HEAD_MAX_E 1024
+__global__ __launch_bounds__(512) void clip_head_kernel(const float* x, long long row_stride, int W, const float* g, const float* b,
+                                                        const float* proj, int E, const float* target, float* feat, float* sim) {
+    __shared__ float cls[LN_MAX_W];
+    __shared__ float fs[HEAD_MAX_E];
+    const int p = blockIdx.x, t = threadIdx.x;
+    if (t < 64) {
+        const float* xr = x + (long long)p * row_stride;
+        ln_row([&](int i) { return xr[i]; }, W, g, b, nullptr, cls);
+    }
+    __syncthreads();
+    for (int n = t; n < E; n += 512) {
+        float acc = 0.f;
+        for (int kk = 0; kk < W; kk += 32) {
+            float w[32];
+#pragma unroll
+            for (int u = 0; u < 32; ++u) w[u] = proj[(long long)(kk + u) * E + n];
+#pragma unroll
+            for (int u = 0; u < 32; ++u) acc = __builtin_fmaf(w[u], cls[kk + u], acc);
+        }
+        const float v = acc + 0.f;
+        feat[(long long)p * E + n] = v;
+        fs[n] = v;
+    }
+    __syncthreads();
+    if (t < 64) cosine_row(fs, target, E, sim + p);
+}
+bool launch_clip_head(const float* x, long long row_stride, int P, int W, const float* g, const float* b, const float* proj, int E,
+                      const float* target, float* feat, float* sim, hipStream_t st) {
+    if (W % 64 != 0 || W > LN_MAX_W || E > HEAD_MAX_E) return false;
+    hipLaunchKernelGGL(clip_head_kernel, dim3(P), dim3(512), 0, st, x, row_stride, W, g, b, proj, E, target, feat, sim);
+    return true;
 }
 void launch_cosine(const float* feat, const float* target, int P, int D, float* sim, hipStream_t st) {
     hipLaunchKernelGGL(cosine_kernel, dim3(P), dim3(64), 0, st, feat, target, D, sim);
diff --git a/clip_glass_amd/csrc/ops.hip b/clip_glass_amd/csrc/ops.hip
--- a/clip_glass_amd/csrc/ops.hip
+++ b/clip_glass_amd/csrc/ops.hip
@@ -190,6 +190,79 @@
     if (rc) return rc;
     if (o16) return down16(out, o16, n);
     GLASS_HIP(hipMemcpy(out, o32, n * sizeof(float), hipMemcpyDeviceToHost));
+    return GLASS_OK;
+}
+
+extern "C" int glass_op_gemm_ln(int32_t device, int32_t M, int32_t N, int32_t K, const float* x32, const float* gamma, const float* beta,
+                                const float* w, const float* bias, int32_t mode, float* out) {
+    OPREQ(x32 && gamma && beta && w && out && (mode == 0 || mode == 1), "bad argument (modes 0 / 1)");
+    OPREQ(K % 64 == 0 && K <= LN_MAX_W, "K must be a multiple of 64, at most 1024");
+    GLASS_HIP(hipSetDevice(device));
+    Dev dv;
+    const size_t n = (size_t)M * N;
+    float* dx = dv.up32(x32, (size_t)M * K);
+    float* st = dv.alloc<float>((size_t)M * (K / LN_BLK) * 2);
+    half_t* o16 = dv.alloc<half_t>(n);
+    launch_row_stats(dx, M, K, st, 0);
+    GemmParams g;
+    memset(&g, 0, sizeof g);
+    g.a32 = dx; g.ln_g = dv.up32(gamma, K); g.ln_b = dv.up32(beta, K); g.ln_stats = st;
+    g.w = dv.up16(w, (size_t)N * K); g.M = M; g.N = N; g.K = K; g.bias = dv.up32(bias, N); g.mode = mode; g.out16 = o16; g.ldo = N;
+    if (!launch_gemm_tiled(g, 0)) { glass_set_error("tiled gemm: shape not covered by the normalising loader"); return GLASS_ERR_ARG; }
+    int rc = finish();
+    if (rc) return rc;
+    return down16(out, o16, n);
+}
+
+extern "C" int glass_op_gemm_stats(int32_t device, int32_t M, int32_t N, int32_t K, int32_t cand_rows, const float* a, const float* w,
+                                   const float* bias, const float* acc, float* out, float* mean_out, float* rstd_out) {
+    OPREQ(a && w && acc && out && mean_out && rstd_out, "null argument");
+    OPREQ(N % 64 == 0 && N <= LN_MAX_W, "N must be a multiple of 64, at most 1024");
+    GLASS_HIP(hipSetDevice(device));
+    Dev dv;
+    const size_t n = (size_t)M * N;
+    GemmParams g;
+    memset(&g, 0, sizeof g);
+    g.a = dv.up16(a, (size_t)M * K); g.w = dv.up16(w, (size_t)N * K); g.M = M; g.N = N; g.K = K; g.bias = dv.up32(bias, N);
+    g.mode = 2; g.out32 = dv.up32(acc, n); g.ldo = N; g.cand_rows = cand_rows;
+    float* st = dv.alloc<float>((size_t)M * (N / LN_BLK) * 2);
+    float* dm = dv.alloc<float>(M);
+    float* dr = dv.alloc<float>(M);
+    g.ln_stats_out = st;
+    if (!launch_gemm_tiled(g, 0)) { glass_set_error("tiled gemm: shape not covered by the statistics epilogue"); return GLASS_ERR_ARG; }
+    launch_ln_stats_combine(st, M, N, dm, dr, 0);
+    int rc = finish();
+    if (rc) return rc;
+    GLASS_HIP(hipMemcpy(out, g.out32, n * sizeof(float), hipMemcpyDeviceToHost));
+    GLASS_HIP(hipMemcpy(mean_out, dm, (size_t)M * sizeof(float), hipMemcpyDeviceToHost));
+    GLASS_HIP(hipMemcpy(rstd_out, dr, (size_t)M * sizeof(float), hipMemcpyDeviceToHost));
+    return GLASS_OK;
+}
+
+extern "C" int glass_op_clip_head(int32_t device, int32_t P, int32_t T, int32_t W, int32_t E, const float* x, const float* gamma,
+                                  const float* beta, const float* proj, const float* target, int32_t fused, float* feat, float* sim) {
+    OPREQ(x && gamma && beta && proj && target && feat && sim && P > 0 && T > 0, "bad argument");
+    GLASS_HIP(hipSetDevice(device));
+    Dev dv;
+    float* dx = dv.up32(x, (size_t)P * T * W);
+    float* dg = dv.up32(gamma, W); float* db = dv.up32(beta, W);
+    float* dp = dv.up32(proj, (size_t)W * E); float* dt = dv.up32(target, E);
+    float* df = dv.alloc<float>((size_t)P * E); float* ds = dv.alloc<float>(P);
+    if (fused) {
+        if (!launch_clip_head(dx, (long long)T * W, P, W, dg, db, dp, E, dt, df, ds, 0)) {
+            glass_set_error("fused head: W must be a multiple of 64, at most 1024, and E at most 1024");
+            return GLASS_ERR_ARG;
+        }
+    } else {
+        float* dc = dv.alloc<float>((size_t)P * W);
+        launch_layernorm(dx, (long long)T * W, P, W, dg, db, nullptr, dc, 0);
+        launch_dense(dc, W, P, W, dp, E, nullptr, df, E, 0, 0, nullptr, 0, 0);
+        launch_cosine(df, dt, P, E, ds, 0);
+    }
+    int rc = finish();
+    if (rc) return rc;
+    GLASS_HIP(hipMemcpy(feat, df, (size_t)P * E * sizeof(float), hipMemcpyDeviceToHost));
+    GLASS_HIP(hipMemcpy(sim, ds, (size_t)P * sizeof(float), hipMemcpyDeviceToHost));
     return GLASS_OK;
 }
 
diff --git a/clip_glass_amd/ops.py b/clip_glass_amd/ops.py
--- a/clip_glass_amd/ops.py
+++ b/clip_glass_amd/ops.py
@@ -113,6 +113,48 @@
     return out
 
 
+def gemm_ln(x32, gamma, beta, w, bias=None, mode=0, device=0):
+    lib = load_library()
+    x32, gamma, beta, w = _f32(x32), _f32(gamma), _f32(beta), _f32(w)
+    M, K = x32.shape
+    N = w.shape[0]
+    out = np.empty((M, N), dtype=np.float32)
+    b, bp = _opt(bias)
+    fp = C.POINTER(C.c_float)
+    lib.glass_op_gemm_ln.argtypes = [C.c_int32] * 4 + [fp] * 5 + [C.c_int32, fp]
+    _check(lib, lib.glass_op_gemm_ln(device, M, N, K, _fp(x32), _fp(gamma), _fp(beta), _fp(w), bp, mode, _fp(out)))
+    return out
+
+
+def gemm_stats(a, w, bias, acc, cand_rows=0, device=0):
+    lib = load_library()
+    a, w, acc = _f32(a), _f32(w), _f32(acc)
+    M, K = a.shape
+    N = w.shape[0]
+    out = np.empty((M, N), dtype=np.float32)
+    mean = np.empty(M, dtype=np.float32)
+    rstd = np.empty(M, dtype=np.float32)
+    b, bp = _opt(bias)
+    fp = C.POINTER(C.c_float)
+    lib.glass_op_gemm_stats.argtypes = [C.c_int32] * 5 + [fp] * 7
+    _check(lib, lib.glass_op_gemm_stats(device, M, N, K, cand_rows, _fp(a), _fp(w), bp, _fp(acc), _fp(out), _fp(mean), _fp(rstd)))
+    return out, mean, rstd
+
+
+def clip_head(x, T, gamma, beta, proj, target, fused=True, device=0):
+    lib = load_library()
+    x, gamma, beta, proj, target = _f32(x), _f32(gamma), _f32(beta), _f32(proj), _f32(target)
+    P, W = x.shape[0] // T, x.shape[1]
+    E = proj.shape[1]
+    feat = np.empty((P, E), dtype=np.float32)
+    sim = np.empty(P, dtype=np.float32)
+    fp = C.POINTER(C.c_float)
+    lib.glass_op_clip_head.argtypes = [C.c_int32] * 5 + [fp] * 5 + [C.c_int32, fp, fp]
+    _check(lib, lib.glass_op_clip_head(device, P, T, W, E, _fp(x), _fp(gamma), _fp(beta), _fp(proj), _fp(target), int(fused),
+                                       _fp(feat), _fp(sim)))
+    return feat, sim
+
+
 def dense(x, wt, bias=None, in_sq=False, mode=0, eps_row=None, device=0):
     lib = load_library()
     x = _f32(x); wt = _f32(wt)
diff --git a/include/glass_ops.h b/include/glass_ops.h
--- a/include/glass_ops.h
+++ b/include/glass_ops.h
@@ -39,6 +39,12 @@
 int glass_op_conv(int32_t device, const glass_conv_desc* d);
 int glass_op_gemm(int32_t device, int32_t M, int32_t N, int32_t K, const float* a, const float* w,
                   const float* bias, int32_t mode, int32_t impl, float* out);
+int glass_op_gemm_ln(int32_t device, int32_t M, int32_t N, int32_t K, const float* x32, const float* gamma, const float* beta,
+                     const float* w, const float* bias, int32_t mode, float* out);
+int glass_op_gemm_stats(int32_t device, int32_t M, int32_t N, int32_t K, int32_t cand_rows, const float* a, const float* w,
+                        const float* bias, const float* acc, float* out, float* mean_out, float* rstd_out);
+int glass_op_clip_head(int32_t device, int32_t P, int32_t T, int32_t W, int32_t E, const float* x, const float* gamma,
+                       const float* beta, const float* proj, const float* target, int32_t fused, float* feat, float* sim);
 int glass_op_dense(int32_t device, int32_t P, int32_t K, int32_t N, const float* x, const float* wt ,
                    const float* bias, int32_t in_sq, int32_t mode, const float* eps_row, float* out);
 int glass_op_torgb(int32_t device, int32_t B, int32_t H, int32_t C, const float* x, const float* wrgb ,
```

Result: no change. 2269 candidates/s (-0.6%).
